# mpeg5/xevd

Hardware: AMD Instinct MI355X
Metric: frames/sec (bit-exact YUV) + achieved HBM GB/s (higher is better)
Workload: dtype s16; 1 GPU; cfg4_main_8k_10b_ra; width=7680, height=4320, bit_depth=10, batches_resident=4, residual_pass_ahead=True, parallelism=1 stream on 1 GPU

## Files before the change

### include/xevd_hip.h

```cpp
#ifndef XEVD_HIP_H
#define XEVD_HIP_H

#include <stddef.h>
#include <stdint.h>

#ifdef __cplusplus
extern "C" {
#endif

#define XGPU_OK                    0
#define XGPU_ERR                  (-1)
#define XGPU_ERR_INVALID_ARGUMENT (-101)
#define XGPU_ERR_OUT_OF_MEMORY    (-102)
#define XGPU_ERR_UNSUPPORTED      (-104)
#define XGPU_ERR_UNEXPECTED       (-105)

#define XGPU_MAX_REFS   17
#define XGPU_PAD_L      144
#define XGPU_PAD_C      72

#define XGPU_MODE_INTRA 0
#define XGPU_MODE_INTER 1
#define XGPU_MODE_SKIP  2
#define XGPU_MODE_DIR   3
// ... 198 lines not shown
int    xgpu_pic_output_device_rois_dev(xgpu_ctx *ctx, int pic, const xgpu_dra_luts *dra, const xgpu_output_format *f, const xgpu_scale_params *sc,
                                       const xgpu_roi_params *rp, const xgpu_roi_bounds *bounds, int box_format, const void *d_boxes, int capacity,
                                       const int *d_count, xgpu_roi_result *d_results, void *d_dst, size_t dst_size, void *stream);
typedef struct xgpu_warp_map { int64_t m[6]; } xgpu_warp_map;
#define XGPU_WARP_CLAMP 0
#define XGPU_WARP_PAD   1
typedef struct xgpu_warp_params { int samples, border; float pad[3]; size_t image_pitch; } xgpu_warp_params;
int    xgpu_warp_from_matrix(const double theta[6], xgpu_warp_map *out);
int    xgpu_warp_from_rotated_box(double cx, double cy, double w, double h, double angle_deg, int dst_w, int dst_h, xgpu_warp_map *out);
int    xgpu_output_warp_check(const xgpu_output_format *f, const xgpu_scale_params *sc, const xgpu_warp_params *wp, const xgpu_warp_map *maps, int n,
                              int width, int height, int bit_depth, int *bad_index);
size_t xgpu_output_warp_size(const xgpu_output_format *f, const xgpu_scale_params *sc, const xgpu_warp_params *wp, int n, int width, int height, int bit_depth);
int    xgpu_pic_output_device_warp(xgpu_ctx *ctx, int pic, const xgpu_dra_luts *dra, const xgpu_output_format *f, const xgpu_scale_params *sc,
                                   const xgpu_warp_params *wp, const xgpu_warp_map *maps, int maps_on_device, int n, int32_t *d_status, void *d_dst,
                                   size_t dst_size, void *stream);
#define XGPU_GRID_Q16_I32 0
#define XGPU_GRID_F32     1
typedef struct xgpu_remap_params { int grid_format, step_log2, samples, border; float pad[3]; size_t grid_pitch, image_pitch; } xgpu_remap_params;
typedef struct xgpu_remap_lens { double fx, fy, cx, cy, k1, k2, p1, p2, k3, nfx, nfy, ncx, ncy; } xgpu_remap_lens;
int    xgpu_remap_grid_dims(int dst_w, int dst_h, int step_log2, int *gw, int *gh);
size_t xgpu_remap_grid_size(const xgpu_scale_params *sc, const xgpu_remap_params *rp, int n);
int    xgpu_output_remap_check(const xgpu_output_format *f, const xgpu_scale_params *sc, const xgpu_remap_params *rp, int n, int width, int height, int bit_depth);
size_t xgpu_output_remap_size(const xgpu_output_format *f, const xgpu_scale_params *sc, const xgpu_remap_params *rp, int n, int width, int height, int bit_depth);
int    xgpu_remap_from_warp(const xgpu_warp_map *map, int dst_w, int dst_h, int step_log2, int32_t *grid);
int    xgpu_remap_from_homography(const double h[9], int dst_w, int dst_h, int step_log2, int32_t *grid);
int    xgpu_remap_from_lens(const xgpu_remap_lens *lens, int dst_w, int dst_h, int step_log2, int32_t *grid);
int    xgpu_pic_output_device_remap(xgpu_ctx *ctx, int pic, const xgpu_dra_luts *dra, const xgpu_output_format *f, const xgpu_scale_params *sc,
                                    const xgpu_remap_params *rp, const void *d_grid, size_t grid_size, int n, void *d_dst, size_t dst_size, void *stream);
#define XGPU_MAX_RUNGS 8
typedef struct xgpu_surface_rung { int width, height; size_t row_pitch; void *d_dst; size_t dst_size; } xgpu_surface_rung;
typedef struct xgpu_ladder_params { int filter; int dst_chroma_loc; } xgpu_ladder_params;
int    xgpu_scale_taps_ex(int n_plane, int subsampling, int siting_half_luma, int n_dst, int dst_subsampling, int dst_siting_half_luma, int filter,
                          int32_t *first, int32_t *count, int16_t *w, int w_stride);
size_t xgpu_output_ladder_rung_size(const xgpu_output_format *f, int rung_width, int rung_height, size_t row_pitch, int bit_depth);
int    xgpu_output_ladder_check(const xgpu_output_format *f, const xgpu_ladder_params *lp, const xgpu_surface_rung *rungs, int n, int width, int height,
                                int bit_depth);
int    xgpu_pic_output_device_ladder(xgpu_ctx *ctx, int pic, const xgpu_dra_luts *dra, const xgpu_output_format *f, const xgpu_ladder_params *lp,
                                     const xgpu_surface_rung *rungs, int n, void *stream);
#define XGPU_SIDE_BLOCKS           0
#define XGPU_SIDE_FLOW_PLANAR      1
#define XGPU_SIDE_FLOW_INTERLEAVED 2
typedef struct xgpu_side_format {
    int layout;
    int dtype;
    int lists;
    int per_poc;
    int crop[4];
    size_t row_pitch;
} xgpu_side_format;
size_t xgpu_side_info_size(const xgpu_side_format *f, int width, int height);
int    xgpu_frame_side_info(xgpu_ctx *ctx, int pic, const xgpu_side_format *f, void *d_dst, size_t dst_size, void *stream);
#define XGPU_RESID_YUV420            0
#define XGPU_RESID_444_PLANAR        1
#define XGPU_RESID_444_INTERLEAVED   2
#define XGPU_RESID_ENERGY            3
typedef struct xgpu_resid_format {
    int layout;
    int dtype;
    int crop[4];
    size_t row_pitch;
} xgpu_resid_format;
size_t xgpu_resid_size(const xgpu_resid_format *f, int width, int height);
int    xgpu_batch_residual(xgpu_ctx *ctx, xgpu_dbatch *db, const xgpu_resid_format *f, void *d_dst, size_t dst_size, void *stream);
#define XGPU_CMP_REF_PIC     0
#define XGPU_CMP_REF_YUV420  1
typedef struct xgpu_compare_ref {
    int kind;
    int pic;
    const void *d_yuv;
    size_t size;
    int dtype;
    size_t row_pitch;
} xgpu_compare_ref;
typedef struct xgpu_compare_params {
    int crop[4];
    int ssim;
    int block_map;
} xgpu_compare_params;
typedef struct xgpu_compare_result {
    uint64_t n[3];
    uint64_t sse[3];
    uint64_t n_diff[3];
    uint64_t first_diff[3];
    uint32_t max_abs[3];
    uint32_t reserved;
    uint64_t ssim_windows[3];
    int64_t  ssim_q30[3];
} xgpu_compare_result;
size_t xgpu_compare_ref_size(const xgpu_compare_ref *r, int width, int height);
size_t xgpu_compare_map_size(const xgpu_compare_params *p, int width, int height);
int    xgpu_compare_check(const xgpu_compare_ref *r, const xgpu_compare_params *p, int width, int height, int bit_depth);
int    xgpu_pic_compare(xgpu_ctx *ctx, int pic, const xgpu_compare_ref *ref, const xgpu_compare_params *p,
                        xgpu_compare_result *d_result, uint64_t *d_map, size_t map_size, void *stream);
typedef struct xgpu_stats_params {
    int crop[4];
    int hist_bits;
    int pctl_e4[2];
    int light;
    int matrix, full_range, chroma_loc, upsample;
    int transfer;
} xgpu_stats_params;
typedef struct xgpu_stats_result {
    uint64_t n[3], sum[3], sum_sq[3];
    uint32_t min[3], max[3];
    uint32_t pctl[3][2];
    uint64_t light_n;
    double   light_sum, light_mean;
    uint32_t light_max_code, light_pctl_code[2], reserved;
    float    light_max, light_pctl[2], reserved2;
} xgpu_stats_result;
size_t xgpu_stats_hist_size(const xgpu_stats_params *p, int bit_depth);
int    xgpu_stats_check(const xgpu_stats_params *p, int width, int height, int bit_depth);
int    xgpu_stats_lin(int transfer, int bit_depth, float lin[4096]);
int    xgpu_pic_stats(xgpu_ctx *ctx, int pic, const xgpu_stats_params *p, xgpu_stats_result *d_result, uint32_t *d_hist, size_t hist_size, void *stream);
int  xgpu_pic_md5(xgpu_ctx *ctx, int pic, const xgpu_dra_luts *dra, uint8_t digest[3][16]);
int  xgpu_pic_download_padded(xgpu_ctx *ctx, int pic, int16_t *buf_y, int16_t *buf_u, int16_t *buf_v);
int  xgpu_pic_upload_padded(xgpu_ctx *ctx, int pic, const int16_t *buf_y, const int16_t *buf_u, const int16_t *buf_v);

int  xgpu_frame_begin(xgpu_ctx *ctx, const xgpu_frame_params *fp);
int  xgpu_batch_create(xgpu_ctx *ctx, const xgpu_cu_batch *b, xgpu_dbatch **out);
int  xgpu_batch_wait_upload(xgpu_ctx *ctx, xgpu_dbatch *db);
int  xgpu_batch_dmvr_mvs(xgpu_ctx *ctx, xgpu_dbatch *db, int16_t *mv, int n);
int  xgpu_set_builder_threads(xgpu_ctx *ctx, int n);
#define XGPU_BATCH_INFO_COUNT 8
int  xgpu_batch_info(xgpu_ctx *ctx, const xgpu_dbatch *db, int info[XGPU_BATCH_INFO_COUNT]);
void xgpu_batch_destroy(xgpu_ctx *ctx, xgpu_dbatch *db);
int  xgpu_batch_prepare(xgpu_ctx *ctx, xgpu_dbatch *db);
int  xgpu_batch_recon(xgpu_ctx *ctx, xgpu_dbatch *db);
int  xgpu_batch_recon_ahead(xgpu_ctx *ctx, xgpu_dbatch *db, xgpu_dbatch *next);
int  xgpu_deblock(xgpu_ctx *ctx);
int  xgpu_alf(xgpu_ctx *ctx, const xgpu_alf_params *ap);
int  xgpu_pad(xgpu_ctx *ctx);
int  xgpu_frame_end(xgpu_ctx *ctx);

enum { XGPU_K_ITDQ = 0, XGPU_K_INTER = 1, XGPU_K_DBK_V = 2, XGPU_K_DBK_H = 3, XGPU_K_PAD = 4, XGPU_K_INTRA = 5,
       XGPU_K_ALF = 6, XGPU_K_AFFINE = 7, XGPU_K_DMVR = 8, XGPU_K_COUNT = 9 };
int  xgpu_timing_enable(xgpu_ctx *ctx, int on);
int  xgpu_timing_reset(xgpu_ctx *ctx);
int  xgpu_timing_get(xgpu_ctx *ctx, double ms[XGPU_K_COUNT], long long launches[XGPU_K_COUNT]);
int  xgpu_measure_copy_bw(xgpu_ctx *ctx, size_t bytes, int iters, double *gbps);

int xgpu_test_mc_l(xgpu_ctx *ctx, const int16_t *ref_plane, int plane_w, int plane_h, int ref_x, int ref_y,
                   int has_dx, int has_dy, int gmv_x, int gmv_y, int16_t *pred, int w, int h, int bit_depth);
int xgpu_test_mc_c(xgpu_ctx *ctx, const int16_t *ref_plane, int plane_w, int plane_h, int ref_x, int ref_y,
                   int has_dx, int has_dy, int gmv_x, int gmv_y, int16_t *pred, int w, int h, int bit_depth);
int xgpu_test_recon(xgpu_ctx *ctx, const int16_t *coef, const int16_t *pred, int is_coef, int cuw, int cuh, int s_rec, int16_t *rec, int bit_depth);
int xgpu_test_dbk(xgpu_ctx *ctx, int16_t *plane, int pw, int ph, int x, int y, int st, int hor, int bit_depth);
int xgpu_test_dbk_chroma(xgpu_ctx *ctx, int16_t *u, int16_t *v, int pw, int ph, int x, int y, int st_u, int st_v, int hor, int bit_depth);
int xgpu_test_batch_resid(xgpu_ctx *ctx, xgpu_dbatch *db, int16_t *resid);
#define XGPU_TEST_BUILD_DIGESTS 13
int xgpu_test_build_batch(const xgpu_seq_params *sp, const xgpu_cu_batch *b, int threads, uint64_t digest[XGPU_TEST_BUILD_DIGESTS], int info[XGPU_BATCH_INFO_COUNT], double *ms);
int xgpu_test_itdq(xgpu_ctx *ctx, int16_t *coef, int n_blocks, int log2w, int log2h, const uint8_t *qp, int bit_depth);
int xgpu_test_itdq_ex(xgpu_ctx *ctx, int16_t *coef, int n_blocks, int log2w, int log2h, const uint8_t *qp, int bit_depth, int tr_v, int tr_h, int log2s);
int xgpu_test_scale_taps_device(xgpu_ctx *ctx, int n_plane, int subsampling, int siting_half_luma, int n_dst, int filter, int32_t *first, int32_t *count,
                                int16_t *w, int w_stride);

#ifdef __cplusplus
}
#endif
#endif
```

### xevd_amd/abi.py

```python
import ctypes as C
import os

import numpy as np

HERE = os.path.dirname(os.path.abspath(__file__))
LIB_PATH = os.path.join(HERE, "libxevd_hip.so")

XGPU_MAX_REFS = 17
PAD_L, PAD_C = 144, 72
MODE_INTRA, MODE_INTER, MODE_SKIP, MODE_DIR = 0, 1, 2, 3
K_NAMES = ["itdq", "inter", "dbk_v", "dbk_h", "pad", "intra", "alf", "affine", "dmvr"]
K_COUNT = 9


class SeqParams(C.Structure):
    _fields_ = [
        ("device", C.c_int), ("width", C.c_int), ("height", C.c_int),
        ("bit_depth_luma", C.c_int), ("bit_depth_chroma", C.c_int), ("chroma_format_idc", C.c_int),
        ("log2_ctu", C.c_int), ("tool_iqt", C.c_int), ("tool_admvp", C.c_int), ("tool_addb", C.c_int),
        ("tool_alf", C.c_int), ("max_pics", C.c_int),
        ("chroma_qp_table", C.POINTER(C.c_int8) * 2),
        ("tool_eipd", C.c_int),
    ]

# ... 561 lines not shown
    cb.pred_mode = _ptr(keep["pred_mode"], C.c_uint8)
    cb.refi, cb.mv = _ptr(keep["refi"], C.c_int8), _ptr(keep["mv"], C.c_int16)
    cb.qp, cb.cbf, cb.ipm = _ptr(keep["qp"], C.c_uint8), _ptr(keep["cbf"], C.c_uint8), _ptr(keep["ipm"], C.c_uint8)
    if keep["cbf_sub"] is not None:
        cb.cbf_sub = _ptr(keep["cbf_sub"], C.c_uint16)
    if keep["ats"] is not None:
        cb.ats = _ptr(keep["ats"], C.c_uint8)
    if keep["ats_inter"] is not None:
        cb.ats_inter = _ptr(keep["ats_inter"], C.c_uint8)
    if keep["affine"] is not None:
        cb.affine, cb.affine_mv = _ptr(keep["affine"], C.c_uint8), _ptr(keep["affine_mv"], C.c_int16)
    if keep["dmvr"] is not None:
        cb.dmvr = _ptr(keep["dmvr"], C.c_uint8)
    if keep["tree"] is not None:
        cb.tree = _ptr(keep["tree"], C.c_uint8)
    cb.coef_off, cb.coef = _ptr(keep["coef_off"], C.c_uint32), _ptr(keep["coef"], C.c_int16)
    cb.n_coef = len(keep["coef"])
    cb.n_ctu = len(keep["ctu_cu_start"]) - 1
    cb.ctu_cu_start = _ptr(keep["ctu_cu_start"], C.c_uint32)
    cb.constrained_intra_pred = int(b.get("constrained_intra_pred", 0) or 0)
    cb.htdf_slice_qp = int(b.get("htdf_slice_qp", 0) or 0)
    if b.get("tiles") is not None:
        keep["tiles"] = make_tile_grid(b["tiles"])
        cb.tiles = C.pointer(keep["tiles"])
    return cb, keep


def make_seq_params(width, height, bit_depth=8, log2_ctu=6, device=0, iqt=0, admvp=0, addb=0, alf=0, max_pics=4,
                    bit_depth_chroma=None, eipd=0):
    sp = SeqParams()
    sp.device, sp.width, sp.height = device, width, height
    sp.bit_depth_luma = bit_depth
    sp.bit_depth_chroma = bit_depth if bit_depth_chroma is None else bit_depth_chroma
    sp.chroma_format_idc = 1
    sp.log2_ctu = log2_ctu
    sp.tool_iqt, sp.tool_admvp, sp.tool_addb, sp.tool_alf = iqt, admvp, addb, alf
    sp.max_pics = max_pics
    sp.tool_eipd = eipd
    return sp


_EXPORTS = {
    "xgpu_open": (C.c_int, [C.POINTER(SeqParams), C.POINTER(C.c_void_p)]),
    "xgpu_close": (None, [C.c_void_p]),
    "xgpu_sync": (C.c_int, [C.c_void_p]),
    "xgpu_last_error": (C.c_char_p, [C.c_void_p]),
    "xgpu_version": (C.c_char_p, []),
    "xgpu_pic_alloc": (C.c_int, [C.c_void_p]),
    "xgpu_pic_free": (C.c_int, [C.c_void_p, C.c_int]),
    "xgpu_pic_upload": (C.c_int, [C.c_void_p, C.c_int, C.c_void_p, C.c_int, C.c_void_p, C.c_void_p, C.c_int]),
    "xgpu_pic_download": (C.c_int, [C.c_void_p, C.c_int, C.c_void_p, C.c_int, C.c_void_p, C.c_void_p, C.c_int]),
    "xgpu_pic_output_size": (C.c_size_t, [C.c_void_p, C.c_int, C.c_int, C.c_int, C.c_int, C.c_int]),
    "xgpu_pic_output": (C.c_int, [C.c_void_p, C.c_int, C.c_void_p, C.c_int, C.c_int, C.c_int, C.c_int, C.c_int, C.c_void_p, C.c_size_t]),
    "xgpu_pic_output_async": (C.c_int, [C.c_void_p, C.c_int, C.c_void_p, C.c_int, C.c_int, C.c_int, C.c_int, C.c_int, C.c_void_p, C.c_size_t, C.POINTER(C.c_int)]),
    "xgpu_pic_output_wait": (C.c_int, [C.c_void_p, C.c_int]),
    "xgpu_pic_md5": (C.c_int, [C.c_void_p, C.c_int, C.c_void_p, C.c_void_p]),
    "xgpu_output_format_size": (C.c_size_t, [C.POINTER(OutputFormat), C.c_int, C.c_int, C.c_int]),
    "xgpu_pic_output_device_size": (C.c_size_t, [C.c_void_p, C.POINTER(OutputFormat)]),
    "xgpu_pic_output_device": (C.c_int, [C.c_void_p, C.c_int, C.c_void_p, C.POINTER(OutputFormat), C.c_void_p, C.c_size_t, C.c_void_p]),
    "xgpu_output_coeffs": (C.c_int, [C.POINTER(OutputFormat), C.c_int, C.POINTER(C.c_int32), C.POINTER(C.c_int), C.POINTER(C.c_float)]),
    "xgpu_colour_tables": (C.c_int, [C.POINTER(OutputFormat), C.POINTER(ColourTransform), C.c_int, C.POINTER(ColourTables)]),
    "xgpu_pic_output_device_cm": (C.c_int, [C.c_void_p, C.c_int, C.c_void_p, C.POINTER(OutputFormat), C.POINTER(ColourTransform), C.c_void_p, C.c_size_t, C.c_void_p]),
    "xgpu_scale_taps": (C.c_int, [C.c_int] * 5 + [C.POINTER(C.c_int32), C.POINTER(C.c_int32), C.POINTER(C.c_int16), C.c_int]),
    "xgpu_output_scaled_size": (C.c_size_t, [C.POINTER(OutputFormat), C.POINTER(ScaleParams), C.c_int, C.c_int, C.c_int]),
    "xgpu_output_scaled_check": (C.c_int, [C.POINTER(OutputFormat), C.POINTER(ScaleParams), C.c_int, C.c_int, C.c_int]),
    "xgpu_pic_output_device_scaled": (C.c_int, [C.c_void_p, C.c_int, C.c_void_p, C.POINTER(OutputFormat), C.POINTER(ScaleParams), C.c_void_p, C.c_size_t, C.c_void_p]),
    "xgpu_scale_taps_ex": (C.c_int, [C.c_int] * 7 + [C.POINTER(C.c_int32), C.POINTER(C.c_int32), C.POINTER(C.c_int16), C.c_int]),
    "xgpu_output_ladder_rung_size": (C.c_size_t, [C.POINTER(OutputFormat), C.c_int, C.c_int, C.c_size_t, C.c_int]),
    "xgpu_output_ladder_check": (C.c_int, [C.POINTER(OutputFormat), C.POINTER(LadderParams), C.POINTER(SurfaceRung), C.c_int, C.c_int, C.c_int, C.c_int]),
    "xgpu_pic_output_device_ladder": (C.c_int, [C.c_void_p, C.c_int, C.c_void_p, C.POINTER(OutputFormat), C.POINTER(LadderParams), C.POINTER(SurfaceRung), C.c_int,
                                                C.c_void_p]),
    "xgpu_roi_inner": (C.c_int, [C.POINTER(Roi), C.POINTER(ScaleParams), C.c_int, C.POINTER(C.c_int)]),
    "xgpu_output_rois_check": (C.c_int, [C.POINTER(OutputFormat), C.POINTER(ScaleParams), C.POINTER(RoiParams), C.POINTER(Roi), C.c_int, C.c_int, C.c_int, C.c_int,
                                         C.POINTER(C.c_int)]),
    "xgpu_output_rois_size": (C.c_size_t, [C.POINTER(OutputFormat), C.POINTER(ScaleParams), C.POINTER(RoiParams), C.POINTER(Roi), C.c_int, C.c_int, C.c_int, C.c_int]),
    "xgpu_pic_output_device_rois": (C.c_int, [C.c_void_p, C.c_int, C.c_void_p, C.POINTER(OutputFormat), C.POINTER(ScaleParams), C.POINTER(RoiParams), C.POINTER(Roi),
                                              C.c_int, C.c_void_p, C.c_size_t, C.c_void_p]),
    "xgpu_output_scaled_cm_check": (C.c_int, [C.POINTER(OutputFormat), C.POINTER(ScaleParams), C.POINTER(ColourTransform), C.c_int, C.c_int, C.c_int]),
    "xgpu_pic_output_device_scaled_cm": (C.c_int, [C.c_void_p, C.c_int, C.c_void_p, C.POINTER(OutputFormat), C.POINTER(ScaleParams), C.POINTER(ColourTransform),
                                                   C.c_void_p, C.c_size_t, C.c_void_p]),
    "xgpu_pic_output_device_rois_cm": (C.c_int, [C.c_void_p, C.c_int, C.c_void_p, C.POINTER(OutputFormat), C.POINTER(ScaleParams), C.POINTER(RoiParams), C.POINTER(Roi),
                                                 C.c_int, C.POINTER(ColourTransform), C.c_void_p, C.c_size_t, C.c_void_p]),
    "xgpu_output_scaled_lin_check": (C.c_int, [C.POINTER(OutputFormat), C.POINTER(ScaleParams), C.POINTER(ColourTransform), C.c_int, C.c_int, C.c_int]),
    "xgpu_output_rois_lin_check": (C.c_int, [C.POINTER(OutputFormat), C.POINTER(ScaleParams), C.POINTER(RoiParams), C.POINTER(Roi), C.c_int, C.POINTER(ColourTransform),
                                             C.c_int, C.c_int, C.c_int, C.POINTER(C.c_int)]),
    "xgpu_pic_output_device_scaled_lin": (C.c_int, [C.c_void_p, C.c_int, C.c_void_p, C.POINTER(OutputFormat), C.POINTER(ScaleParams), C.POINTER(ColourTransform),
                                                    C.c_void_p, C.c_size_t, C.c_void_p]),
    "xgpu_pic_output_device_rois_lin": (C.c_int, [C.c_void_p, C.c_int, C.c_void_p, C.POINTER(OutputFormat), C.POINTER(ScaleParams), C.POINTER(RoiParams), C.POINTER(Roi),
                                                  C.c_int, C.POINTER(ColourTransform), C.c_void_p, C.c_size_t, C.c_void_p]),
    "xgpu_roi_snap": (C.c_int, [C.c_int, C.c_void_p, C.c_int, C.c_int, C.POINTER(Roi)]),
    "xgpu_output_rois_dev_check": (C.c_int, [C.POINTER(OutputFormat), C.POINTER(ScaleParams), C.POINTER(RoiParams), C.POINTER(RoiBounds)] + [C.c_int] * 5),
    "xgpu_output_rois_dev_size": (C.c_size_t, [C.POINTER(OutputFormat), C.POINTER(ScaleParams), C.POINTER(RoiParams), C.POINTER(RoiBounds)] + [C.c_int] * 5),
    "xgpu_pic_output_device_rois_dev": (C.c_int, [C.c_void_p, C.c_int, C.c_void_p, C.POINTER(OutputFormat), C.POINTER(ScaleParams), C.POINTER(RoiParams),
                                                  C.POINTER(RoiBounds), C.c_int, C.c_void_p, C.c_int, C.c_void_p, C.c_void_p, C.c_void_p, C.c_size_t, C.c_void_p]),
    "xgpu_warp_from_matrix": (C.c_int, [C.POINTER(C.c_double), C.POINTER(WarpMap)]),
    "xgpu_warp_from_rotated_box": (C.c_int, [C.c_double] * 5 + [C.c_int, C.c_int, C.POINTER(WarpMap)]),
    "xgpu_output_warp_check": (C.c_int, [C.POINTER(OutputFormat), C.POINTER(ScaleParams), C.POINTER(WarpParams), C.POINTER(WarpMap), C.c_int, C.c_int, C.c_int, C.c_int,
                                         C.POINTER(C.c_int)]),
    "xgpu_output_warp_size": (C.c_size_t, [C.POINTER(OutputFormat), C.POINTER(ScaleParams), C.POINTER(WarpParams), C.c_int, C.c_int, C.c_int, C.c_int]),
    "xgpu_pic_output_device_warp": (C.c_int, [C.c_void_p, C.c_int, C.c_void_p, C.POINTER(OutputFormat), C.POINTER(ScaleParams), C.POINTER(WarpParams), C.c_void_p,
                                              C.c_int, C.c_int, C.c_void_p, C.c_void_p, C.c_size_t, C.c_void_p]),
    "xgpu_remap_grid_dims": (C.c_int, [C.c_int, C.c_int, C.c_int, C.POINTER(C.c_int), C.POINTER(C.c_int)]),
    "xgpu_remap_grid_size": (C.c_size_t, [C.POINTER(ScaleParams), C.POINTER(RemapParams), C.c_int]),
    "xgpu_output_remap_check": (C.c_int, [C.POINTER(OutputFormat), C.POINTER(ScaleParams), C.POINTER(RemapParams), C.c_int, C.c_int, C.c_int, C.c_int]),
    "xgpu_output_remap_size": (C.c_size_t, [C.POINTER(OutputFormat), C.POINTER(ScaleParams), C.POINTER(RemapParams), C.c_int, C.c_int, C.c_int, C.c_int]),
    "xgpu_remap_from_warp": (C.c_int, [C.POINTER(WarpMap), C.c_int, C.c_int, C.c_int, C.POINTER(C.c_int32)]),
    "xgpu_remap_from_homography": (C.c_int, [C.POINTER(C.c_double), C.c_int, C.c_int, C.c_int, C.POINTER(C.c_int32)]),
    "xgpu_remap_from_lens": (C.c_int, [C.POINTER(RemapLens), C.c_int, C.c_int, C.c_int, C.POINTER(C.c_int32)]),
    "xgpu_pic_output_device_remap": (C.c_int, [C.c_void_p, C.c_int, C.c_void_p, C.POINTER(OutputFormat), C.POINTER(ScaleParams), C.POINTER(RemapParams), C.c_void_p,
                                               C.c_size_t, C.c_int, C.c_void_p, C.c_size_t, C.c_void_p]),
    "xgpu_side_info_size": (C.c_size_t, [C.POINTER(SideFormat), C.c_int, C.c_int]),
    "xgpu_frame_side_info": (C.c_int, [C.c_void_p, C.c_int, C.POINTER(SideFormat), C.c_void_p, C.c_size_t, C.c_void_p]),
    "xgpu_resid_size": (C.c_size_t, [C.POINTER(ResidFormat), C.c_int, C.c_int]),
    "xgpu_batch_residual": (C.c_int, [C.c_void_p, C.c_void_p, C.POINTER(ResidFormat), C.c_void_p, C.c_size_t, C.c_void_p]),
    "xgpu_compare_ref_size": (C.c_size_t, [C.POINTER(CompareRef), C.c_int, C.c_int]),
    "xgpu_compare_map_size": (C.c_size_t, [C.POINTER(CompareParams), C.c_int, C.c_int]),
    "xgpu_compare_check": (C.c_int, [C.POINTER(CompareRef), C.POINTER(CompareParams), C.c_int, C.c_int, C.c_int]),
    "xgpu_pic_compare": (C.c_int, [C.c_void_p, C.c_int, C.POINTER(CompareRef), C.POINTER(CompareParams), C.c_void_p, C.c_void_p, C.c_size_t, C.c_void_p]),
    "xgpu_stats_hist_size": (C.c_size_t, [C.POINTER(StatsParams), C.c_int]),
    "xgpu_stats_check": (C.c_int, [C.POINTER(StatsParams), C.c_int, C.c_int, C.c_int]),
    "xgpu_stats_lin": (C.c_int, [C.c_int, C.c_int, C.POINTER(C.c_float)]),
    "xgpu_pic_stats": (C.c_int, [C.c_void_p, C.c_int, C.POINTER(StatsParams), C.c_void_p, C.c_void_p, C.c_size_t, C.c_void_p]),
    "xgpu_host_alloc": (C.c_int, [C.c_void_p, C.c_size_t, C.POINTER(C.c_void_p)]),
    "xgpu_host_free": (None, [C.c_void_p, C.c_void_p]),
    "xgpu_batch_wait_upload": (C.c_int, [C.c_void_p, C.c_void_p]),
    "xgpu_set_builder_threads": (C.c_int, [C.c_void_p, C.c_int]),
    "xgpu_batch_prepare": (C.c_int, [C.c_void_p, C.c_void_p]),
    "xgpu_batch_info": (C.c_int, [C.c_void_p, C.c_void_p, C.POINTER(C.c_int)]),
    "xgpu_batch_dmvr_mvs": (C.c_int, [C.c_void_p, C.c_void_p, C.c_void_p, C.c_int]),
    "xgpu_pic_download_padded": (C.c_int, [C.c_void_p, C.c_int, C.c_void_p, C.c_void_p, C.c_void_p]),
    "xgpu_pic_upload_padded": (C.c_int, [C.c_void_p, C.c_int, C.c_void_p, C.c_void_p, C.c_void_p]),
    "xgpu_frame_begin": (C.c_int, [C.c_void_p, C.POINTER(FrameParams)]),
    "xgpu_batch_create": (C.c_int, [C.c_void_p, C.POINTER(CuBatch), C.POINTER(C.c_void_p)]),
    "xgpu_batch_destroy": (None, [C.c_void_p, C.c_void_p]),
    "xgpu_batch_recon": (C.c_int, [C.c_void_p, C.c_void_p]),
    "xgpu_batch_recon_ahead": (C.c_int, [C.c_void_p, C.c_void_p, C.c_void_p]),
    "xgpu_deblock": (C.c_int, [C.c_void_p]),
    "xgpu_alf": (C.c_int, [C.c_void_p, C.POINTER(AlfParams)]),
    "xgpu_pad": (C.c_int, [C.c_void_p]),
    "xgpu_frame_end": (C.c_int, [C.c_void_p]),
    "xgpu_timing_enable": (C.c_int, [C.c_void_p, C.c_int]),
    "xgpu_timing_reset": (C.c_int, [C.c_void_p]),
    "xgpu_timing_get": (C.c_int, [C.c_void_p, C.POINTER(C.c_double), C.POINTER(C.c_longlong)]),
    "xgpu_measure_copy_bw": (C.c_int, [C.c_void_p, C.c_size_t, C.c_int, C.POINTER(C.c_double)]),
    "xgpu_test_mc_l": (C.c_int, [C.c_void_p, C.c_void_p] + [C.c_int] * 8 + [C.c_void_p] + [C.c_int] * 3),
    "xgpu_test_mc_c": (C.c_int, [C.c_void_p, C.c_void_p] + [C.c_int] * 8 + [C.c_void_p] + [C.c_int] * 3),
    "xgpu_test_batch_resid": (C.c_int, [C.c_void_p, C.c_void_p, C.c_void_p]),
    "xgpu_test_build_batch": (C.c_int, [C.c_void_p, C.c_void_p, C.c_int, C.POINTER(C.c_uint64), C.POINTER(C.c_int), C.POINTER(C.c_double)]),
    "xgpu_test_recon": (C.c_int, [C.c_void_p, C.c_void_p, C.c_void_p] + [C.c_int] * 4 + [C.c_void_p, C.c_int]),
    "xgpu_test_dbk": (C.c_int, [C.c_void_p, C.c_void_p] + [C.c_int] * 7),
    "xgpu_test_dbk_chroma": (C.c_int, [C.c_void_p, C.c_void_p, C.c_void_p] + [C.c_int] * 8),
    "xgpu_test_itdq": (C.c_int, [C.c_void_p, C.c_void_p, C.c_int, C.c_int, C.c_int, C.c_void_p, C.c_int]),
    "xgpu_test_itdq_ex": (C.c_int, [C.c_void_p, C.c_void_p, C.c_int, C.c_int, C.c_int, C.c_void_p, C.c_int, C.c_int, C.c_int, C.c_int]),
    "xgpu_test_scale_taps_device": (C.c_int, [C.c_void_p] + [C.c_int] * 5 + [C.POINTER(C.c_int32), C.POINTER(C.c_int32), C.POINTER(C.c_int16), C.c_int]),
}

_lib = None


def exported_names():
    return sorted(_EXPORTS)


def _share_torch_hip_runtime():
    import importlib.util
    import sys
    if "torch" in sys.modules:
        return
    spec = importlib.util.find_spec("torch")
    if spec is None or not spec.submodule_search_locations:
        return
    rt = os.path.join(list(spec.submodule_search_locations)[0], "lib", "libamdhip64.so")
    if os.path.exists(rt):
        C.CDLL(rt, mode=C.RTLD_GLOBAL)


def load():
    global _lib
    if _lib is None:
        _share_torch_hip_runtime()
        if not os.path.exists(LIB_PATH):
            raise RuntimeError(
                f"{LIB_PATH} is missing: build it with `python -c 'import __graft_entry__ as g; g.build()'` "
                "(hipcc --offload-arch=gfx950).  xevd_amd has no CPU fallback.")
        lib = C.CDLL(LIB_PATH)
        for name, (res, args) in _EXPORTS.items():
            fn = getattr(lib, name)
            fn.restype, fn.argtypes = res, args
        _lib = lib
    return _lib
```

### xevd_amd/csrc/itdq_body.h

```cpp
#pragma once
#include "xgpu_internal.h"
#include <type_traits>

typedef short v2s __attribute__((ext_vector_type(2)));

static __constant__ uint32_t k_tmp[2730];
__host__ __device__ constexpr int tmp_base(int log2n) { return log2n == 1 ? 0 : log2n == 2 ? 2 : log2n == 3 ? 10 : log2n == 4 ? 42 : log2n == 5 ? 170 : 682; }

static __constant__ uint32_t k_atsp[2][680];
__host__ __device__ constexpr int atsp_base(int log2n) { return log2n == 2 ? 0 : log2n == 3 ? 8 : log2n == 4 ? 40 : 168; }

static void upload_transform_tables_tu(const int *tm, const int16_t *ats, hipStream_t s)
{
    static uint32_t apk[2][680];
    for (int t = 0; t < 2; t++) {
        int src = 0;
        for (int l = 2; l <= 5; l++) {
            const int N = 1 << l, dst = atsp_base(l);
            for (int k2 = 0; k2 < N / 2; k2++)
                for (int n = 0; n < N; n++)
                    apk[t][dst + k2 * N + n] = (uint32_t)(uint16_t)ats[t * 1360 + src + (2 * k2) * N + n] |
                                               ((uint32_t)(uint16_t)ats[t * 1360 + src + (2 * k2 + 1) * N + n] << 16);
            src += N * N;
        }
    }
    (void)hipMemcpyToSymbolAsync(HIP_SYMBOL(k_atsp), apk, sizeof(apk), 0, hipMemcpyHostToDevice, s);
    static uint32_t packed[2730];
    int src = 0;
    for (int l = 1; l <= 6; l++) {
        const int N = 1 << l, dst = tmp_base(l);
        for (int k2 = 0; k2 < N / 2; k2++)
            for (int n = 0; n < N; n++)
                packed[dst + k2 * N + n] = (uint32_t)(uint16_t)(int16_t)tm[src + (2 * k2) * N + n] |
                                           ((uint32_t)(uint16_t)(int16_t)tm[src + (2 * k2 + 1) * N + n] << 16);
        src += N * N;
    }
    (void)hipMemcpyToSymbolAsync(HIP_SYMBOL(k_tmp), packed, sizeof(packed), 0, hipMemcpyHostToDevice, s);
    (void)hipStreamSynchronize(s);
}

__device__ __forceinline__ int clip16(int v) { return min(max(v, -32768), 32767); }
__device__ __forceinline__ int dot2(uint32_t a, uint32_t b, int c)
{
    return __builtin_amdgcn_sdot2(__builtin_bit_cast(v2s, a), __builtin_bit_cast(v2s, b), c, false);
}
__device__ __forceinline__ int mad24(int a, int b, int c)
{
    int r;
    asm("v_mad_i32_i24 %0, %1, %2, %3" : "=v"(r) : "v"(a), "v"(b), "v"(c));
    return r;
}
__device__ __forceinline__ uint32_t pack16(int lo, int hi) { return (uint32_t)(uint16_t)lo | ((uint32_t)hi << 16); }

__host__ __device__ constexpr int itdq_group(int lw, int lh)
{
    const int W = 1 << lw, H = 1 << lh;
    const int l1 = W * (H > 16 ? H / 16 : 1), l2 = H * (W > 16 ? W / 16 : 1);
    return 256 / (l1 > l2 ? l1 : l2);
}

#define ITDQ_PLANES_DWORDS 4608
#define ITDQ_LDS_DWORDS (ITDQ_PLANES_DWORDS + 2048)
#define ITDQ_MAX_G 32
#define ITDQ_TB_DWORDS (4 * ITDQ_MAX_G)

typedef uint32_t itq_v2 __attribute__((ext_vector_type(2)));
typedef uint32_t itq_v4 __attribute__((ext_vector_type(4)));
typedef itq_v2 __attribute__((aligned(4))) itq_v2_u;
typedef itq_v4 __attribute__((aligned(2))) itq_v4_u;
typedef itq_v2 __attribute__((aligned(2))) itq_v2_s;
template <typename T> __device__ __forceinline__ T itq_any() { T v; asm volatile("" : "=v"(v)); return v; }
static_assert(sizeof(TbRec) == 8, "a TbRec is fetched as one 8-byte load: off | log2w, log2h, qp, log2s");
__device__ __forceinline__ void itq_rec_if(itq_v2 &v, const TbRec *p, bool on) { if (on) v = *(const itq_v2_u *)p; }
__device__ __forceinline__ int rec_qp(itq_v2 r) { return (int)((r.y >> 16) & 0xFF); }
__device__ __forceinline__ int rec_log2s(itq_v2 r) { return (int)(r.y >> 24); }

template <bool ODD, bool IQT>
struct ItdqScale {
    int mul, cmax, shift, offset;
    __device__ __forceinline__ ItdqScale(int qp, int bd, int lwh)
    {
        shift = bd - 9 + (lwh >> 1) + (ODD ? 8 : 0);
        offset = shift == 0 ? 0 : 1 << (shift - 1);
        const int q6 = (int)(((uint32_t)qp * 171u) >> 10), sidx = qp - 6 * q6;
        constexpr uint64_t scale = 40ull | 45ull << 8 | 51ull << 16 | 57ull << 24 | 64ull << 32 | (uint64_t)(IQT ? 72 : 71) << 40;
        const int sbase = (int)((scale >> (8 * sidx)) & 0xFF);
        mul = sbase << q6;
        cmax = (1 << 23) >> q6;
    }
    __device__ __forceinline__ int operator()(int c) const
    {
        if constexpr (!ODD) {
            const int held = min(max(c, -cmax), cmax);
            return clip16(mad24(held, mul, offset) >> shift);
        }
        const long long l = ((long long)(c * (ODD ? 181 : 1)) * mul + offset) >> shift;
        return (int)min(max(l, -32768ll), 32767ll);
    }
};

template <int G, int LX>
__device__ __forceinline__ uint32_t wave_masks(const uint32_t *s_m, int t)
{
    constexpr int X = 1 << LX, PER = 64 / X > 1 ? 64 / X : 1, N = G < PER ? G : PER;
    const int p0 = __builtin_amdgcn_readfirstlane(((t & ~63) % (G * X)) >> LX);
    static_assert(G * X >= 64 ? (G % N == 0) : (64 % (G * X) == 0 && N == G), "the wave's TBs are entries [p0, p0 + N)");
    uint32_t m = 0;
#pragma unroll
    for (int i = 0; i < N; i++) m |= s_m[p0 + i];
    return (uint32_t)__builtin_amdgcn_readfirstlane((int)m);
}

template <int L>
__device__ __forceinline__ const uint32_t *itdq_matrix(int tr) { return (tr == TR_DCT2 || L < 2 || L > 5) ? k_tmp + tmp_base(L) : k_atsp[tr - 1] + atsp_base(L); }

template <int LW, int LH, bool IQT>
__device__ __forceinline__ void itdq_small(const ItdqArgs &a, const TbWave wv)
{
    constexpr int W = 1 << LW, H = 1 << LH, S = W * H;
    static_assert(S <= 16 && itdq_group(LW, LH) <= 256, "one TB per lane");
    const int p = threadIdx.x;
    if (p >= wv.count) return;
    const itq_v2 rec = *(const itq_v2_u *)(a.tbs + wv.first + p);
    const uint32_t *tmh = itdq_matrix<LH>(wv.tr_v), *tmw = itdq_matrix<LW>(wv.tr_h);
    const bool s16_mid = IQT || wv.tr_v != TR_DCT2 || wv.tr_h != TR_DCT2;
    uint32_t raw[S / 2];
    if constexpr (S == 4) { const itq_v2 v = *(const itq_v2_s *)(a.coef + rec.x); raw[0] = v.x; raw[1] = v.y; }
    else {
#pragma unroll
        for (int i = 0; i < S / 8; i++) {
            const itq_v4 v = *(const itq_v4_u *)(a.coef + rec.x + 8 * i);
            raw[4 * i] = v.x; raw[4 * i + 1] = v.y; raw[4 * i + 2] = v.z; raw[4 * i + 3] = v.w;
        }
    }
    const ItdqScale<(LW + LH) & 1, IQT> dq(rec_qp(rec), a.bd, LW + LH);
    int d[S];
#pragma unroll
    for (int i = 0; i < S / 2; i++) {
        d[2 * i] = 0; d[2 * i + 1] = 0;
        if (raw[i] != 0) { d[2 * i] = dq((int16_t)(raw[i] & 0xFFFF)); d[2 * i + 1] = dq((int16_t)(raw[i] >> 16)); }
    }
    uint32_t mh[H][W / 2], ml[H][W / 2];
#pragma unroll
    for (int jj = 0; jj < W / 2; jj++) {
        int acc[2][H];
#pragma unroll
        for (int e = 0; e < 2; e++) {
#pragma unroll
            for (int n = 0; n < H; n++) acc[e][n] = 0;
#pragma unroll
            for (int k2 = 0; k2 < H / 2; k2++) {
                const uint32_t vp = pack16(d[(2 * k2) * W + 2 * jj + e], d[(2 * k2 + 1) * W + 2 * jj + e]);
#pragma unroll
                for (int n = 0; n < H; n++) acc[e][n] = dot2(tmh[k2 * H + n], vp, acc[e][n]);
            }
        }
#pragma unroll
        for (int n = 0; n < H; n++) {
            if (s16_mid) mh[n][jj] = pack16(clip16((acc[0][n] + 64) >> 7), clip16((acc[1][n] + 64) >> 7));
            else if constexpr (!IQT) {
                mh[n][jj] = pack16(acc[0][n] >> 15, acc[1][n] >> 15);
                ml[n][jj] = pack16(acc[0][n] & 0x7FFF, acc[1][n] & 0x7FFF);
            }
        }
    }
    const int shift2 = s16_mid ? 12 - (a.bd - 8) : 7 + 12 - (a.bd - 8);
    uint32_t out[S / 2];
#pragma unroll
    for (int r = 0; r < H; r++) {
        int res[W];
        if (s16_mid) {
            int s[W];
#pragma unroll
            for (int n = 0; n < W; n++) s[n] = 1 << (shift2 - 1);
#pragma unroll
            for (int k2 = 0; k2 < W / 2; k2++) {
#pragma unroll
                for (int n = 0; n < W; n++) s[n] = dot2(tmw[k2 * W + n], mh[r][k2], s[n]);
            }
#pragma unroll
            for (int n = 0; n < W; n++) res[n] = clip16(s[n] >> shift2);
        } else if constexpr (!IQT) {
            int sh[W], sl[W];
#pragma unroll
            for (int n = 0; n < W; n++) { sh[n] = 0; sl[n] = 0; }
#pragma unroll
            for (int k2 = 0; k2 < W / 2; k2++) {
#pragma unroll
                for (int n = 0; n < W; n++) { sh[n] = dot2(tmw[k2 * W + n], mh[r][k2], sh[n]); sl[n] = dot2(tmw[k2 * W + n], ml[r][k2], sl[n]); }
            }
            const long long add = 1ll << (shift2 - 1);
#pragma unroll
            for (int n = 0; n < W; n++) {
                const long long s = (long long)sh[n] * 32768 + sl[n] + add;
                res[n] = (int)min(max(s >> shift2, -32768ll), 32767ll);
            }
        }
#pragma unroll
        for (int n = 0; n < W; n += 2) out[(r * W + n) / 2] = pack16(res[n], res[n + 1]);
    }
    int16_t *dst = a.resid + rec.x;
    if constexpr (S == 4) { itq_v2 v; v.x = out[0]; v.y = out[1]; *(itq_v2_s *)dst = v; }
    else {
#pragma unroll
        for (int i = 0; i < S / 8; i++) {
            itq_v4 v; v.x = out[4 * i]; v.y = out[4 * i + 1]; v.z = out[4 * i + 2]; v.w = out[4 * i + 3];
            *(itq_v4_u *)(dst + 8 * i) = v;
        }
    }
}

template <int LW, int LH, bool IQT>
__device__ __forceinline__ void itdq_item(const ItdqArgs &a, const TbWave wv, uint32_t *lds, uint32_t *s_tb)
{
    constexpr int W = 1 << LW, H = 1 << LH;
    constexpr int N1 = H > 16 ? 16 : H, C1 = H / N1;
    constexpr int N2 = W > 16 ? 16 : W, C2 = W / N2;
    constexpr int G = itdq_group(LW, LH);
    constexpr int RS = W / 2 + 1;
    constexpr int PLANE = G * H * RS;
    constexpr bool UNI1 = (G * W) % 64 == 0, UNI2 = (G * H) % 64 == 0;
    static_assert(2 * PLANE <= ITDQ_PLANES_DWORDS && G * W * H <= 4096 && G <= ITDQ_MAX_G, "LDS budget");
    constexpr int PLANES_DWORDS = IQT ? ITDQ_PLANES_DWORDS / 2 : ITDQ_PLANES_DWORDS;
    constexpr bool RMASK = H >= 16, CMASK = W >= 16;
    uint32_t *s_rm = s_tb, *s_cm = s_tb + ITDQ_MAX_G, *s_rec = s_tb + 2 * ITDQ_MAX_G;
    const int t = threadIdx.x;

    constexpr int S = W * H, UN = S >= 8 ? 8 : 4, NU = G * S / UN, NR = (NU + 255) / 256;
    typedef typename std::conditional<UN == 8, itq_v4, itq_v2>::type cvec;
    bool on[NR];
    int up[NR], uo[NR];
    itq_v2 rec[NR];
#pragma unroll
    for (int r = 0; r < NR; r++) {
        const int u = t + 256 * r;
        up[r] = (u * UN) / S; uo[r] = (u * UN) % S;
        on[r] = (NU % 256 == 0 || u < NU) && up[r] < wv.count;
        rec[r] = itq_any<itq_v2>();
        itq_rec_if(rec[r], a.tbs + wv.first + up[r], on[r]);
    }
    if (RMASK || CMASK) {
        if (t < G) { s_rm[t] = 0; s_cm[t] = 0; }
        __syncthreads();
    }
    const uint32_t *tmh = itdq_matrix<LH>(wv.tr_v), *tmw = itdq_matrix<LW>(wv.tr_h);
    const bool s16_mid = IQT || wv.tr_v != TR_DCT2 || wv.tr_h != TR_DCT2;
    asm volatile("" :: "s"(tmh), "s"(tmw));
    int16_t *ldsh = (int16_t *)lds;
    int16_t *ldsl = (int16_t *)(lds + PLANE);
    uint32_t *ldsc = lds + PLANES_DWORDS;
    cvec cv[NR];
#pragma unroll
    for (int r = 0; r < NR; r++) {
        cv[r] = itq_any<cvec>();
        if (on[r]) {
            const int16_t *src = a.coef + rec[r].x + ((uo[r] >> LW) << rec_log2s(rec[r])) + (uo[r] & (W - 1));
            if constexpr (UN == 8) cv[r] = *(const itq_v4_u *)src; else cv[r] = *(const itq_v2_s *)src;
        }
    }
#pragma unroll
    for (int r = 0; r < NR; r++) {
        if (!on[r]) continue;
        const int p = up[r], o = uo[r];
        const ItdqScale<(LW + LH) & 1, IQT> dq(rec_qp(rec[r]), a.bd, LW + LH);
        if (o == 0) { s_rec[2 * p] = rec[r].x; s_rec[2 * p + 1] = rec[r].y; }
        uint32_t raw[UN / 2];
#pragma unroll
        for (int i = 0; i < UN / 2; i++) raw[i] = cv[r][i];
#pragma unroll
        for (int i = 0; i < UN / 2; i++) {
            if (raw[i] == 0) continue;
            raw[i] = pack16(dq((int16_t)(raw[i] & 0xFFFF)), dq((int16_t)(raw[i] >> 16)));
            if (RMASK) atomicOr(&s_rm[p], 1u << ((o + 2 * i) >> (LW + 1)));
            if (CMASK) atomicOr(&s_cm[p], 1u << (((o + 2 * i) & (W - 1)) >> 1));
        }
#pragma unroll
        for (int i = 0; i < UN / 2; i++) ldsc[(p * S + o) / 2 + i] = raw[i];
    }
    __syncthreads();

    uint32_t rows1 = 0;
    if (RMASK) rows1 = wave_masks<G, LW>(s_rm, t);
    if (t < G * W * C1) {
        const int idx = t % (G * W);
        int chunk = t / (G * W);
        if (UNI1) chunk = __builtin_amdgcn_readfirstlane(chunk);
        const int p = idx >> LW, j = idx & (W - 1);
        const bool valid = p < wv.count;
        const uint32_t vmask = valid ? 0xFFFFFFFFu : 0u;
        const int16_t *src = (const int16_t *)ldsc + p * (W * H) + j;

        int acc[N1];
#pragma unroll
        for (int n = 0; n < N1; n++) acc[n] = 0;
        if (RMASK) {
            for (uint32_t m = rows1; m; m &= m - 1) {
                const int k2 = __builtin_ctz(m);
                const uint32_t vp = pack16(src[(2 * k2) * W], src[(2 * k2 + 1) * W]) & vmask;
                const uint32_t *row = tmh + k2 * H + chunk * N1;
#pragma unroll
                for (int n = 0; n < N1; n++) acc[n] = dot2(row[n], vp, acc[n]);
            }
        } else {
            for (int k2 = 0; k2 < H / 2; k2++) {
                const uint32_t vp = pack16(src[(2 * k2) * W], src[(2 * k2 + 1) * W]) & vmask;
                if (__ballot(vp != 0) == 0) continue;
                const uint32_t *row = tmh + k2 * H + chunk * N1;
#pragma unroll
                for (int n = 0; n < N1; n++) acc[n] = dot2(row[n], vp, acc[n]);
            }
        }
        const int base = (p * H + chunk * N1) * (2 * RS) + j;
        if (CMASK && !(valid && ((s_cm[p] >> (j >> 1)) & 1))) {
        } else if (s16_mid) {
#pragma unroll
            for (int n = 0; n < N1; n++) ldsh[base + n * (2 * RS)] = (int16_t)clip16((acc[n] + 64) >> 7);
        } else {
#pragma unroll
            for (int n = 0; n < N1; n++) {
                ldsh[base + n * (2 * RS)] = (int16_t)(acc[n] >> 15);
                ldsl[base + n * (2 * RS)] = (int16_t)(acc[n] & 0x7FFF);
            }
        }
    }
    __syncthreads();

    uint32_t cols2 = 0;
    if (CMASK) cols2 = wave_masks<G, LH>(s_cm, t);
    if (t < G * H * C2) {
        const int idx = t % (G * H);
        int chunk = t / (G * H);
        if (UNI2) chunk = __builtin_amdgcn_readfirstlane(chunk);
        const int p = idx >> LH, r = idx & (H - 1);
        if (p >= wv.count) return;
        const uint32_t own = CMASK ? s_cm[p] : 0xFFFFFFFFu;
        itq_v2 tb;
        tb.x = s_rec[2 * p]; tb.y = s_rec[2 * p + 1];
        const int shift2 = s16_mid ? 12 - (a.bd - 8) : 7 + 12 - (a.bd - 8);
        const uint32_t *inh = lds + (p * H + r) * RS;
        const uint32_t *inl = inh + PLANE;
        int res[N2];
        if (s16_mid) {
            int s[N2];
#pragma unroll
            for (int n = 0; n < N2; n++) s[n] = 1 << (shift2 - 1);
            if (CMASK) {
                for (uint32_t m = cols2; m; m &= m - 1) {
                    const int k2 = __builtin_ctz(m);
                    const uint32_t vp = inh[k2] & (0u - ((own >> k2) & 1));
                    const uint32_t *row = tmw + k2 * W + chunk * N2;
#pragma unroll
                    for (int n = 0; n < N2; n++) s[n] = dot2(row[n], vp, s[n]);
                }
            } else {
                for (int k2 = 0; k2 < W / 2; k2++) {
                    const uint32_t vp = inh[k2];
                    if (__ballot(vp != 0) == 0) continue;
                    const uint32_t *row = tmw + k2 * W + chunk * N2;
#pragma unroll
                    for (int n = 0; n < N2; n++) s[n] = dot2(row[n], vp, s[n]);
                }
            }
#pragma unroll
            for (int n = 0; n < N2; n++) res[n] = clip16(s[n] >> shift2);
        } else {
            int sh[N2], sl[N2];
#pragma unroll
            for (int n = 0; n < N2; n++) { sh[n] = 0; sl[n] = 0; }
            if (CMASK) {
                for (uint32_t m = cols2; m; m &= m - 1) {
                    const int k2 = __builtin_ctz(m);
                    const uint32_t mine = 0u - ((own >> k2) & 1);
                    const uint32_t vh = inh[k2] & mine, vl = inl[k2] & mine;
                    const uint32_t *row = tmw + k2 * W + chunk * N2;
#pragma unroll
                    for (int n = 0; n < N2; n++) { sh[n] = dot2(row[n], vh, sh[n]); sl[n] = dot2(row[n], vl, sl[n]); }
                }
            } else {
                for (int k2 = 0; k2 < W / 2; k2++) {
                    const uint32_t vh = inh[k2], vl = inl[k2];
                    if (__ballot((vh | vl) != 0) == 0) continue;
                    const uint32_t *row = tmw + k2 * W + chunk * N2;
#pragma unroll
                    for (int n = 0; n < N2; n++) { sh[n] = dot2(row[n], vh, sh[n]); sl[n] = dot2(row[n], vl, sl[n]); }
                }
            }
            const long long add = 1ll << (shift2 - 1);
#pragma unroll
            for (int n = 0; n < N2; n++) {
                const long long s = (long long)sh[n] * 32768 + sl[n] + add;
                res[n] = (int)min(max(s >> shift2, -32768ll), 32767ll);
            }
        }
        int16_t *out = a.resid + tb.x + (r << rec_log2s(tb)) + chunk * N2;
        if constexpr (N2 >= 8) {
#pragma unroll
            for (int n = 0; n < N2; n += 8) {
                uint4 v;
                v.x = pack16(res[n + 0], res[n + 1]);
                v.y = pack16(res[n + 2], res[n + 3]);
                v.z = pack16(res[n + 4], res[n + 5]);
                v.w = pack16(res[n + 6], res[n + 7]);
                *(uint4 *)(out + n) = v;
            }
        } else if constexpr (N2 == 4) {
            uint2 v;
            v.x = pack16(res[0], res[1]);
            v.y = pack16(res[2], res[3]);
            *(uint2 *)out = v;
        } else {
            *(uint32_t *)out = pack16(res[0], res[1]);
        }
    }
}

template <bool IQT>
__device__ __forceinline__ void itdq_dispatch(const ItdqArgs &a, int wi, uint32_t *lds, uint32_t *s_tb)
{
    static_assert(sizeof(TbWave) == 12 && alignof(TbWave) == 4, "TbWave is read as three dwords");
    const uint32_t *w = (const uint32_t *)(a.waves + wi);
    const uint32_t w0 = w[0], w1 = w[1], w2 = w[2];
    TbWave wv;
    wv.first = w0; wv.count = (uint16_t)(w1 & 0xFFFF); wv.log2w = (uint8_t)(w1 >> 16); wv.log2h = (uint8_t)(w1 >> 24); wv.tr_v = (uint8_t)w2; wv.tr_h = (uint8_t)(w2 >> 8);
#define CASE(lw, lh) case (lw) * 8 + (lh): if constexpr ((lw) + (lh) <= 4) itdq_small<lw, lh, IQT>(a, wv); else itdq_item<lw, lh, IQT>(a, wv, lds, s_tb); break;
#define ROW(lw) CASE(lw, 1) CASE(lw, 2) CASE(lw, 3) CASE(lw, 4) CASE(lw, 5) CASE(lw, 6)
    switch (wv.log2w * 8 + wv.log2h) {
        ROW(1) ROW(2) ROW(3) ROW(4) ROW(5) ROW(6)
        default: break;
    }
#undef ROW
#undef CASE
}
```

### xevd_amd/csrc/k_intra.hip

```cpp
#include "xgpu_internal.h"
#include "itdq_body.h"

#include <type_traits>
#include "intra_pred.h"

#define INTRA_WAVES 8


__constant__ uint8_t k_htdf_tbl[5][16] = {
    { 0, 0, 2,  6, 10, 14, 19, 23, 28, 32,  36,  41,  45,  49,  53,  57 },
    { 0, 0, 5, 12, 20, 29, 38, 47, 56, 65,  73,  82,  90,  98, 107, 115 },
    { 0, 0, 1,  4,  9, 16, 24, 32, 41, 50,  59,  68,  77,  86,  94, 103 },
    { 0, 0, 3,  9, 19, 32, 47, 64, 81, 99, 117, 135, 154, 179, 205, 230 },
    { 0, 0, 0,  2,  6, 11, 18, 27, 38, 51,  64,  96, 128, 160, 192, 224 },
};
#define HTDF_EXT (66 * 66)

template <bool HTDF> struct IntraLds { static constexpr int WAVE = (HTDF && HTDF_EXT > 3 * NB_LEN) ? HTDF_EXT : 3 * NB_LEN; };

#ifdef INTRA_PROFILE
__device__ uint32_t g_intra_prof[8 * 64];
#define ISTAMP(k) do { if (DEP && t == 0 && item >= INTRA_PROFILE && item < INTRA_PROFILE + 64) g_intra_prof[8 * (item - INTRA_PROFILE) + (k)] = (uint32_t)clock64(); } while (0)
#else
#define ISTAMP(k)
// ... 462 lines not shown
            else                 filter_tiles(std::integral_constant<int, 2>{}, std::integral_constant<int, 2>{});
        }
        ISTAMP(4);
        if (DEP) {
            asm volatile("s_waitcnt vmcnt(0)" ::: "memory");
            ISTAMP(5);
            if (t == 0) __hip_atomic_store(&a.done[item], a.epoch, __ATOMIC_RELAXED, __HIP_MEMORY_SCOPE_AGENT);
        }
        wave_lds_sync();
        if (!DEP) break;
        item = uni(q0.x);
        if (item == 0xFFFFFFFFu) break;
    }
}

#define SB_C0 71
#define SB_UR 144
#define SB_LEN (SB_UR + 72)
#define SMALL_GROUPS (4 * INTRA_WAVES)
__device__ __forceinline__ void intra_small_body(const IntraArgs &a, uint32_t block, int16_t *s_nb_)
{
    int16_t (*s_nb)[3][SB_LEN] = (int16_t (*)[3][SB_LEN])s_nb_;
    const int g = threadIdx.x >> 4, t = threadIdx.x & 15;
    const uint32_t k = block * SMALL_GROUPS + (uint32_t)g;
    if (k >= (uint32_t)a.n_small) return;
    const uint32_t item = (uint32_t)(a.first + a.count - a.n_small) + k;
    int16_t (*nb)[SB_LEN] = s_nb[g];
    const int mid = 1 << (a.bd_l - 1), maxv = (1 << a.bd_l) - 1;
    const uint4 *rec = (const uint4 *)&a.list[item];
    const uint4 q0 = rec[0], q1 = rec[1], q2 = rec[2];
    const uint32_t nflags = q0.y, avail_ul = nflags & 1;
    const int lrf = (int)((nflags >> 23) & 3);
    const uint64_t avail_up = (uint64_t)q0.z | ((lrf & 2) ? 0ull : (uint64_t)q0.w << 32);
    const uint64_t avail_le = (uint64_t)q1.x | ((uint64_t)q1.y << 32);
    const uint32_t gg = q2.x, m = q2.y, ipm = q2.z, coef_off = q2.w;
    const int cu_x = gg & 0xFFFF, cu_y = gg >> 16;
    const int lw = m & 0xFF, lh = (m >> 8) & 0xFF, cbf = (m >> 16) & 0xFF;
    const int mode_l = ipm & 0xFF, mode_c = (ipm >> 8) & 0xFF;
    const int cw = 1 << lw, chh = 1 << lh, scuw = cw >> 2, nscu = scuw * (chh >> 2), cwc = cw >> 1;
    const uint32_t off_u = coef_off + ((cbf & 1) ? (uint32_t)(cw * chh) : 0u);
    const uint32_t off_v = off_u + ((cbf & 2) ? (uint32_t)(cwc * (chh >> 1)) : 0u);
    const bool has = t < nscu;
    const int lx = (t & (scuw - 1)) << 2, ly = (t >> (lw - 2)) << 2;

    uint2 rl[4] = { { 0, 0 }, { 0, 0 }, { 0, 0 }, { 0, 0 } };
    uint32_t rc[2][2] = { { 0, 0 }, { 0, 0 } };
    if (has) {
        if (cbf & 1)
#pragma unroll
            for (int r = 0; r < 4; r++) rl[r] = *(const uint2 *)(a.resid + coef_off + (ly + r) * cw + lx);
#pragma unroll
        for (int c = 1; c < 3; c++)
            if ((cbf >> c) & 1)
#pragma unroll
                for (int r = 0; r < 2; r++) rc[c - 1][r] = *(const uint32_t *)(a.resid + (c == 1 ? off_u : off_v) + ((ly >> 1) + r) * cwc + (lx >> 1));
    }

#pragma unroll
    for (int c = 0; c < 3; c++) {
        const int16_t *plane = c == 0 ? a.cur_y : (c == 1 ? a.cur_u : a.cur_v);
        const int s = c ? a.s_c : a.s_l, sh = c ? 1 : 0, ush = c ? 1 : 2;
        const int16_t *org = plane + (cu_y >> sh) * s + (cu_x >> sh);
        const int n = (cw + chh) >> sh;
        const int eu = min(2 * t, n - 2), e0 = min(t, n - 1), e1 = min(t + 16, n - 1);
        const uint32_t vu = *(const uint32_t *)(org - s + eu);
        const uint32_t v0 = (uint16_t)org[e0 * s - 1], v1 = (uint16_t)org[e1 * s - 1], vc = (uint16_t)org[-s - 1];
        const uint32_t midp = (uint32_t)mid * 0x10001u;
        if (2 * t < n) *(uint32_t *)&nb[c][SB_C0 + 1 + 2 * t] = ((avail_up >> (eu >> ush)) & 1) ? vu : midp;
        if (t < n) nb[c][SB_C0 - 1 - t] = (int16_t)(((avail_le >> (e0 >> ush)) & 1) ? v0 : (uint32_t)mid);
        if (t + 16 < n) nb[c][SB_C0 - 1 - (t + 16)] = (int16_t)(((avail_le >> (e1 >> ush)) & 1) ? v1 : (uint32_t)mid);
        if (t == 0) nb[c][SB_C0] = (int16_t)(avail_ul ? vc : (uint32_t)mid);
        if (n > 32) {
            for (int e = 2 * t + 32; e < n; e += 32)
                *(uint32_t *)&nb[c][SB_C0 + 1 + e] = ((avail_up >> (e >> ush)) & 1) ? *(const uint32_t *)(org - s + e) : midp;
            for (int e = t + 32; e < n; e += 16)
                nb[c][SB_C0 - 1 - e] = ((avail_le >> (e >> ush)) & 1) ? org[e * s - 1] : (int16_t)mid;
        }
    }
    wave_lds_sync();
#pragma unroll
    for (int c = 0; c < 3; c++) {
        const int mode = c ? mode_c : mode_l;
        const int w = c ? cw >> 1 : cw, h = c ? chh >> 1 : chh;
        if (mode == 0) {
            int acc = 0;
            for (int e = t; e < w + h; e += 16) acc += e < h ? nb[c][SB_C0 - 1 - e] : nb[c][SB_C0 + 1 + e - h];
            acc = row_sum16(acc);
            if (t == 0) nb[c][NB_DC] = (int16_t)((acc + w) >> ((c ? lw - 1 : lw) + 1));
        } else if (mode == 4) {
            for (int e = t; e < w + h; e += 16) nb[c][SB_UR + e] = (int16_t)((nb[c][SB_C0 + 1 + e] + nb[c][SB_C0 - 1 - e]) >> 1);
        }
    }
    wave_lds_sync();
    if (!has) return;
    const int x = cu_x + lx, y = cu_y + ly;
    int pl[4][4], pc[2][2][2];
    int vl[7], vc[2][3];
    nb_fetch<7, SB_C0, SB_UR>(nb[0], mode_l, lx, ly, vl);
    nb_fetch<3, SB_C0, SB_UR>(nb[1], mode_c, lx >> 1, ly >> 1, vc[0]);
    nb_fetch<3, SB_C0, SB_UR>(nb[2], mode_c, lx >> 1, ly >> 1, vc[1]);
#pragma unroll
    for (int md = 0; md < 5; md++) {
        if (md == mode_l)
#pragma unroll
            for (int r = 0; r < 4; r++)
#pragma unroll
                for (int q = 0; q < 4; q++) pl[r][q] = vl[nb_sel(md, r, q, 3)];
        if (md == mode_c)
#pragma unroll
            for (int c = 0; c < 2; c++)
#pragma unroll
                for (int r = 0; r < 2; r++)
#pragma unroll
                    for (int q = 0; q < 2; q++) pc[c][r][q] = vc[c][nb_sel(md, r, q, 1)];
    }
    int16_t *dy = a.cur_y + y * a.s_l + x;
    const int coff = (y >> 1) * a.s_c + (x >> 1);
    if (!(nflags & 32u))
#pragma unroll
        for (int r = 0; r < 4; r++) {
            const uint32_t o0 = recon2i(pack2i(pl[r][0], pl[r][1]), (cbf & 1) ? rl[r].x : 0u, maxv), o1 = recon2i(pack2i(pl[r][2], pl[r][3]), (cbf & 1) ? rl[r].y : 0u, maxv);
            *(uint2 *)(dy + r * a.s_l) = make_uint2(o0, o1);
        }
    if (!(nflags & 64u))
#pragma unroll
        for (int c = 1; c < 3; c++) {
            int16_t *d = (c == 1 ? a.cur_u : a.cur_v) + coff;
#pragma unroll
            for (int r = 0; r < 2; r++)
                *(uint32_t *)(d + r * a.s_c) = recon2i(pack2i(pc[c - 1][r][0], pc[c - 1][r][1]), ((cbf >> c) & 1) ? rc[c - 1][r] : 0u, maxv);
        }
}

__global__ __launch_bounds__(64 * INTRA_WAVES) void k_intra_l1(const IntraArgs a, uint32_t big)
{
    constexpr int BIG_LDS = INTRA_WAVES * IntraLds<false>::WAVE, SMALL_LDS = SMALL_GROUPS * 3 * SB_LEN;
    __shared__ __attribute__((aligned(16))) int16_t s_nb[BIG_LDS > SMALL_LDS ? BIG_LDS : SMALL_LDS];
    if (blockIdx.x < big) {
        IntraArgs b = a;
        b.count = a.count - a.n_small;
        intra_body<false, 0, false, false, INTRA_WAVES>(b, blockIdx.x, s_nb, nullptr);
    } else intra_small_body(a, blockIdx.x - big, s_nb);
}

template <bool DEP, int EIPD, bool IBC, bool HTDF>
__global__ __launch_bounds__(64 * INTRA_WAVES) void k_intra(const IntraArgs a)
{
    __shared__ __attribute__((aligned(16))) int16_t s_nb[INTRA_WAVES * IntraLds<HTDF>::WAVE];
    __shared__ uint32_t s_chunk;
    intra_body<DEP, EIPD, IBC, HTDF, INTRA_WAVES>(a, blockIdx.x, s_nb, &s_chunk);
}

#define FUSED_WAVES 4
template <int EIPD, bool IBC, bool IQT>
__global__ __launch_bounds__(64 * FUSED_WAVES) void k_intra_itdq(const IntraArgs a, const ItdqArgs r, uint32_t n_intra_wg, uint64_t rate)
{
    constexpr int ITDQ_DW = (IQT ? ITDQ_LDS_DWORDS - ITDQ_PLANES_DWORDS / 2 : ITDQ_LDS_DWORDS) + ITDQ_TB_DWORDS, INTRA_DW = (FUSED_WAVES * IntraLds<false>::WAVE + 1) / 2 + 4;
    __shared__ __attribute__((aligned(16))) uint32_t raw[ITDQ_DW > INTRA_DW ? ITDQ_DW : INTRA_DW];
    const uint32_t before = min(n_intra_wg, (uint32_t)(((uint64_t)blockIdx.x * rate) >> 32)), after = min(n_intra_wg, (uint32_t)(((uint64_t)(blockIdx.x + 1) * rate) >> 32));
    if (after > before) {
        intra_body<true, EIPD, IBC, false, FUSED_WAVES>(a, blockIdx.x, (int16_t *)raw, raw + INTRA_DW - 1);
    } else {
        const int wi = (int)(blockIdx.x - before);
        if (wi >= r.n_waves) return;
        itdq_dispatch<IQT>(r, wi, raw, raw + ITDQ_DW - ITDQ_TB_DWORDS);
    }
}

void upload_transform_tables_intra(const int *tm, const int16_t *ats, hipStream_t s) { upload_transform_tables_tu(tm, ats, s); }

int intra_chunk(bool with_itdq) { return with_itdq ? FUSED_WAVES : INTRA_WAVES; }

void launch_intra(xgpu_ctx *c, const IntraArgs &a, bool dep, bool ibc, bool htdf, const ItdqArgs *next, bool right)
{
    right = right && c->sp.tool_eipd;
    if (next) {
        const uint32_t n_wg = (uint32_t)((a.count + FUSED_WAVES - 1) / FUSED_WAVES);
        const dim3 g(n_wg + (uint32_t)next->n_waves), b(64 * FUSED_WAVES);
        const uint32_t span = std::max(n_wg, g.x / 2);
        const uint64_t rate = (((uint64_t)n_wg << 32) + span - 1) / span;
#define LAUNCHF(E, I) do { if (next->iqt) hipLaunchKernelGGL((k_intra_itdq<E, I, true>), g, b, 0, c->stream, a, *next, n_wg, rate); else hipLaunchKernelGGL((k_intra_itdq<E, I, false>), g, b, 0, c->stream, a, *next, n_wg, rate); } while (0)
        if (right) LAUNCHF(2, true);
        else if (c->sp.tool_eipd) { if (ibc) LAUNCHF(1, true); else LAUNCHF(1, false); }
        else                 { if (ibc) LAUNCHF(0, true); else LAUNCHF(0, false); }
#undef LAUNCHF
        return;
    }
    const int per = INTRA_WAVES;
    if (!dep && !right && !htdf && !ibc && !c->sp.tool_eipd && a.n_small >= c->intra_small_min) {
        const uint32_t big = (uint32_t)((a.count - a.n_small + per - 1) / per), small_blocks = (uint32_t)((a.n_small + SMALL_GROUPS - 1) / SMALL_GROUPS);
        hipLaunchKernelGGL(k_intra_l1, dim3(big + small_blocks), dim3(64 * INTRA_WAVES), 0, c->stream, a, big);
        return;
    }
    const int blocks = (a.count + per - 1) / per;
    const dim3 g(blocks), b(64 * INTRA_WAVES);
#define LAUNCH(D, E, I, H) hipLaunchKernelGGL((k_intra<D, E, I, H>), g, b, 0, c->stream, a)
    if (right) { if (dep) LAUNCH(true, 2, true, true); else LAUNCH(false, 2, true, true); }
    else if (htdf) {
        if (c->sp.tool_eipd) { if (dep) LAUNCH(true, 1, true, true); else LAUNCH(false, 1, true, true); }
        else                 { if (dep) LAUNCH(true, 0, true, true); else LAUNCH(false, 0, true, true); }
    } else if (ibc) {
        if (c->sp.tool_eipd) { if (dep) LAUNCH(true, 1, true, false); else LAUNCH(false, 1, true, false); }
        else                 { if (dep) LAUNCH(true, 0, true, false); else LAUNCH(false, 0, true, false); }
    } else {
        if (c->sp.tool_eipd) { if (dep) LAUNCH(true, 1, false, false); else LAUNCH(false, 1, false, false); }
        else                 { if (dep) LAUNCH(true, 0, false, false); else LAUNCH(false, 0, false, false); }
    }
#undef LAUNCH
#ifdef INTRA_PROFILE
    static int shots = 0;
    if (dep && ++shots == 5) {
        hipStreamSynchronize(c->stream);
        uint32_t h[8 * 64];
        hipMemcpyFromSymbol(h, HIP_SYMBOL(g_intra_prof), sizeof(h));
        for (int i = 0; i < 64; i++)
            fprintf(stderr, "  pos %d start %10u  wait %6u stage %5u (EIPD luma: issue %5u, return %5u | HTDF: to the block loads %5u from stamp 3, block in LDS %5u) plan %5u predict %5u ack %5u\n", INTRA_PROFILE + i, h[8 * i], h[8 * i + 1] - h[8 * i],
                    h[8 * i + 2] - h[8 * i + 1], h[8 * i + 6] - h[8 * i + 1], h[8 * i + 7] - h[8 * i + 6], h[8 * i + 6] - h[8 * i + 3], h[8 * i + 7] - h[8 * i + 6], h[8 * i + 3] - h[8 * i + 2], h[8 * i + 4] - h[8 * i + 3], h[8 * i + 5] - h[8 * i + 4]);
    }
#endif
}
```

### xevd_amd/csrc/xgpu_api.hip

```cpp
#include "xgpu_host.h"

static const int8_t k_chroma_qp_main[58] = { 0, 1, 2, 3, 4, 5, 6, 7, 8, 9, 10, 11, 12, 13, 14, 15, 16, 17, 18, 19, 20, 21, 22, 23, 24, 25, 26, 27, 28, 29,
    29, 30, 31, 32, 33, 34, 35, 36, 37, 37, 38, 39, 40, 40, 41, 42, 43, 44, 45, 46, 47, 48, 49, 50, 51, 52, 53, 54 };
static const int8_t k_chroma_qp_base[58] = {
     0,  1,  2,  3,  4,  5,  6,  7,  8,  9, 10, 11, 12, 13, 14, 15, 16, 17, 18, 19,
    20, 21, 22, 23, 24, 25, 26, 27, 28, 29, 29, 29, 30, 31, 32, 32, 33, 33, 34, 34,
    35, 35, 36, 36, 36, 37, 37, 37, 38, 38, 39, 39, 40, 40, 40, 41, 41, 41 };


const char *xgpu_version(void) { return "xevd_amd 0.1 (gfx950)"; }
const char *xgpu_last_error(const xgpu_ctx *c) { return c ? c->err : "null ctx"; }

void time_begin(xgpu_ctx *c, int k, hipEvent_t *a, hipEvent_t *b)
{
    if (!c->timing) return;
    auto get = [&]() {
        hipEvent_t e;
        if (!c->ev_pool.empty()) { e = c->ev_pool.back(); c->ev_pool.pop_back(); }
        else (void)hipEventCreate(&e);
        return e;
    };
    *a = get(); *b = get();
    (void)hipEventRecord(*a, c->stream);
    (void)k;
}
void time_end(xgpu_ctx *c, int k, hipEvent_t a, hipEvent_t b)
{
    if (!c->timing) return;
    (void)hipEventRecord(b, c->stream);
    c->ev_pending.push_back({ a, b, k });
}
int xgpu_timing_enable(xgpu_ctx *c, int on) { ARGCHK(c, c != NULL); c->timing = on; return XGPU_OK; }
int xgpu_timing_reset(xgpu_ctx *c)
{
    ARGCHK(c, c != NULL);
    HIPCHK(c, hipStreamSynchronize(c->stream));
    for (auto &e : c->ev_pending) { c->ev_pool.push_back(e.a); c->ev_pool.push_back(e.b); }
    c->ev_pending.clear();
    memset(c->t_ms, 0, sizeof(c->t_ms));
    memset(c->t_n, 0, sizeof(c->t_n));
    return XGPU_OK;
}
int xgpu_timing_get(xgpu_ctx *c, double ms[XGPU_K_COUNT], long long n[XGPU_K_COUNT])
{
    ARGCHK(c, c != NULL);
    HIPCHK(c, hipStreamSynchronize(c->stream));
    for (auto &e : c->ev_pending) {
        float t = 0;
        HIPCHK(c, hipEventElapsedTime(&t, e.a, e.b));
        c->t_ms[e.k] += t; c->t_n[e.k]++;
        c->ev_pool.push_back(e.a); c->ev_pool.push_back(e.b);
    }
    c->ev_pending.clear();
    for (int i = 0; i < XGPU_K_COUNT; i++) { ms[i] = c->t_ms[i]; n[i] = c->t_n[i]; }
    return XGPU_OK;
}

static void init_transform_tables(xgpu_ctx *c)
{
    static int tm[5460];
    int o = 0;
    for (int l = 1; l <= 6; l++) {
        const int N = 1 << l;
        for (int k = 0; k < N; k++)
            for (int n = 0; n < N; n++) {
                const double v = k == 0 ? 64.0 : 64.0 * sqrt(2.0) * cos((2 * n + 1) * k * 3.14159265358979323846 / (2.0 * N));
                tm[o++] = (int)(v >= 0 ? floor(v + 0.5) : -floor(-v + 0.5));
            }
    }
    static int16_t ats[2 * 1360];
    for (int t = 0; t < 2; t++) {
        int q = t * 1360;
        for (int l = 2; l <= 5; l++) {
            const int N = 1 << l;
            const double sc = sqrt((double)N) * 64;
            int16_t m[32 * 32];
            for (int k = 0; k < N; k++)
                for (int n = 0; n < N; n++) {
                    const double v = t == 0 ? sin(3.14159265358979323846 * (k + 0.5) * (n + 1) / (N + 0.5)) * sqrt(2.0 / (N + 0.5))
                                            : cos(3.14159265358979323846 * (k + 0.5) * (n + 0.5) / (N + 0.5)) * sqrt(2.0 / (N + 0.5));
                    m[k * N + n] = (int16_t)(sc * v + (v > 0 ? 0.5 : -0.5));
                }
            if (N == 4) {
                const int a = m[0], b = m[1], cc = m[2], d = m[3];
                const int e7[16] = { a, b, cc, b + a,  cc, cc, 0, -cc,  a + b, -a, -cc, b,  b, -(b + a), cc, -a };
                const int e8[16] = { d + cc, b, cc, d,  b, 0, -b, -b,  cc, -b, -d, d + cc,  d, -b, d + cc, -cc };
                for (int i = 0; i < 16; i++) m[i] = (int16_t)(t == 0 ? e7[i] : e8[i]);
            }
            for (int i = 0; i < N * N; i++) ats[q++] = m[i];
        }
    }
    upload_transform_tables(tm, ats, c->stream);
}

int xgpu_open(const xgpu_seq_params *sp, xgpu_ctx **out)
{
    if (!sp || !out) return XGPU_ERR_INVALID_ARGUMENT;
    *out = NULL;
    if (sp->chroma_format_idc != 1) return XGPU_ERR_UNSUPPORTED;
    if (sp->width <= 0 || sp->height <= 0 || (sp->width & 7) || (sp->height & 7)) return XGPU_ERR_INVALID_ARGUMENT;
    if (sp->bit_depth_luma < 8 || sp->bit_depth_luma > 12 || sp->bit_depth_chroma < 8 || sp->bit_depth_chroma > 12) return XGPU_ERR_UNSUPPORTED;
    if (sp->log2_ctu < 5 || sp->log2_ctu > 7) return XGPU_ERR_INVALID_ARGUMENT;
    int ndev = 0;
    if (hipGetDeviceCount(&ndev) != hipSuccess || ndev <= 0 || sp->device < 0 || sp->device >= ndev) return XGPU_ERR_UNEXPECTED;

    xgpu_ctx *c = new xgpu_ctx();
    c->sp = *sp;
    c->sp.chroma_qp_table[0] = c->sp.chroma_qp_table[1] = NULL;
    c->builder_threads = 1;
    c->err[0] = 0; c->timing = 0; c->have_frame = 0; c->side_pic = -1; c->d_maps = NULL; c->d_dra = NULL; c->d_cm = NULL; c->cm_tab = NULL; c->d_ctb_flag = NULL; c->stream = 0; c->up_stream = 0; c->down_stream = 0; c->side_stream = 0; c->after_inter = 0; c->have_after_inter = 0; c->where = 0; c->addb_pending = 0;
    c->fork_ev = c->join_ev = 0;
    c->intra_small_min = getenv("XEVD_HIP_INTRA_SMALL_MIN") ? std::max(1, atoi(getenv("XEVD_HIP_INTRA_SMALL_MIN"))) : 2048;
    c->addb_scalar = getenv("XEVD_HIP_ADDB_SCALAR") != NULL;
    c->dmvr_scalar = getenv("XEVD_HIP_DMVR_SCALAR") != NULL;
    c->split_addb_alf = getenv("XEVD_HIP_SPLIT_ADDB_ALF") != NULL;
    for (int i = 0; i < 2; i++) { c->d_out[i] = NULL; c->out_caps[i] = 0; c->out_ready[i] = c->out_done[i] = 0; c->out_busy[i] = 0; }
    c->d_md5 = NULL; c->md5_ready = 0;
    c->odev_ev[0] = c->odev_ev[1] = 0;
    c->sc_tab = NULL; c->sc_tab_cap = 0; c->sc_mid = NULL; c->sc_mid_cap = 0; c->cmp_part = NULL; c->cmp_part_cap = 0; c->stats_blk = NULL; c->stats_lin_tc = c->stats_lin_bd = -1;
    c->roi_blk = NULL; c->roi_blk_cap = 0;
    c->lad_blk = NULL; c->lad_blk_cap = 0; c->lad_cap = 0;
    for (int i = 0; i < 6; i++) c->sc_key[i] = -1;
    c->out_next = 0;
    memset(c->t_ms, 0, sizeof(c->t_ms)); memset(c->t_n, 0, sizeof(c->t_n));
    const int boff = 6 * (sp->bit_depth_chroma - 8);
    for (int t = 0; t < 2; t++)
        for (int q = -boff; q <= 57; q++)
            c->chroma_qp[t][q + boff] = sp->chroma_qp_table[t] ? sp->chroma_qp_table[t][q + boff] : (int8_t)(q < 0 ? q : (sp->tool_iqt ? k_chroma_qp_main[q] : k_chroma_qp_base[q]));

    auto fail = [&](int code) { xgpu_close(c); return code; };
    if (hipSetDevice(sp->device) != hipSuccess) return fail(XGPU_ERR_UNEXPECTED);
    static const bool blocking = getenv("XEVD_HIP_BLOCKING_SYNC") != NULL && atoi(getenv("XEVD_HIP_BLOCKING_SYNC")) != 0;
    if (blocking) (void)hipSetDeviceFlags(hipDeviceScheduleBlockingSync);
    const unsigned ev_flags = hipEventDisableTiming | (blocking ? hipEventBlockingSync : 0);
    {
        static std::atomic<int> n_ctx(0);
        static const bool no_rot = getenv("XEVD_HIP_NO_QUEUE_ROTATION") != NULL;
        const bool swap = !no_rot && (n_ctx.fetch_add(1) & 1);
        hipStream_t *const order[4] = { swap ? &c->side_stream : &c->stream, &c->up_stream, &c->down_stream, swap ? &c->stream : &c->side_stream };
        for (int i = 0; i < 4; i++)
            if (hipStreamCreateWithFlags(order[i], hipStreamNonBlocking) != hipSuccess) return fail(XGPU_ERR_UNEXPECTED);
    }
    if (hipEventCreateWithFlags(&c->after_inter, hipEventDisableTiming) != hipSuccess) return fail(XGPU_ERR_UNEXPECTED);
    if (hipEventCreateWithFlags(&c->fork_ev, hipEventDisableTiming) != hipSuccess || hipEventCreateWithFlags(&c->join_ev, hipEventDisableTiming) != hipSuccess) return fail(XGPU_ERR_UNEXPECTED);
    for (int i = 0; i < 2; i++)
        if (hipEventCreateWithFlags(&c->out_ready[i], hipEventDisableTiming) != hipSuccess || hipEventCreateWithFlags(&c->out_done[i], ev_flags) != hipSuccess)
            return fail(XGPU_ERR_UNEXPECTED);

    ctx_geometry(c);

    if (hipMalloc((void **)&c->d_maps, sizeof(ScuRec) * (size_t)c->w_scu * c->h_scu) != hipSuccess) return fail(XGPU_ERR_OUT_OF_MEMORY);
    if (hipMemsetAsync(c->d_maps, 0, sizeof(ScuRec) * (size_t)c->w_scu * c->h_scu, c->stream) != hipSuccess) return fail(XGPU_ERR_UNEXPECTED);
    if (hipMalloc((void **)&c->d_ctb_flag, (size_t)c->w_ctu * c->h_ctu + 16) != hipSuccess) return fail(XGPU_ERR_OUT_OF_MEMORY);
    init_transform_tables(c);
    c->pics.resize(1 + std::max(1, std::min(sp->max_pics, 34)));
    for (auto &p : c->pics) { p.base = NULL; p.used = 0; }
    {
        DevPic &p = c->pics[0];
        if (hipMalloc((void **)&p.base, c->pic_elems * sizeof(int16_t)) != hipSuccess) return fail(XGPU_ERR_OUT_OF_MEMORY);
        (void)hipMemsetAsync(p.base, 0, c->pic_elems * sizeof(int16_t), c->stream);
        p.s_l = c->s_l; p.s_c = c->s_c; p.used = 1;
        p.y = p.base + (size_t)XGPU_PAD_L * c->s_l + XGPU_MARGIN_L;
        p.u = p.base + c->off_u + (size_t)XGPU_PAD_C * c->s_c + XGPU_MARGIN_C;
        p.v = p.base + c->off_v + (size_t)XGPU_PAD_C * c->s_c + XGPU_MARGIN_C;
    }
    if (hipStreamSynchronize(c->stream) != hipSuccess) return fail(XGPU_ERR_UNEXPECTED);
    *out = c;
    return XGPU_OK;
}

void xgpu_close(xgpu_ctx *c)
{
    if (!c) return;
    (void)hipSetDevice(c->sp.device);
    if (c->stream) (void)hipStreamSynchronize(c->stream);
    if (c->up_stream) (void)hipStreamSynchronize(c->up_stream);
    if (c->down_stream) (void)hipStreamSynchronize(c->down_stream);
    if (c->side_stream) (void)hipStreamSynchronize(c->side_stream);
    for (auto &p : c->pics) if (p.base) (void)hipFree(p.base);
    if (c->d_maps) (void)hipFree(c->d_maps);
    for (BatchBlock &k : c->pool) block_free(k);
    for (auto &h : c->pinned) (void)hipHostFree(h.p);
    c->pinned.clear();
    c->pool.clear();
    if (c->d_md5) (void)hipFree(c->d_md5);
    if (c->md5_ready) (void)hipEventDestroy(c->md5_ready);
    for (int i = 0; i < 2; i++) if (c->odev_ev[i]) (void)hipEventDestroy(c->odev_ev[i]);
    for (int i = 0; i < 2; i++) { if (c->d_out[i]) (void)hipFree(c->d_out[i]); if (c->out_ready[i]) (void)hipEventDestroy(c->out_ready[i]); if (c->out_done[i]) (void)hipEventDestroy(c->out_done[i]); }
    if (c->d_dra) (void)hipFree(c->d_dra);
    if (c->d_cm) (void)hipFree(c->d_cm);
    delete c->cm_tab;
    if (c->sc_tab) (void)hipFree(c->sc_tab);
    if (c->sc_mid) (void)hipFree(c->sc_mid);
    if (c->cmp_part) (void)hipFree(c->cmp_part);
    if (c->stats_blk) (void)hipFree(c->stats_blk);
    if (c->roi_blk) (void)hipFree(c->roi_blk);
    if (c->lad_blk) (void)hipFree(c->lad_blk);
    if (c->d_ctb_flag) (void)hipFree(c->d_ctb_flag);
    for (auto &e : c->ev_pending) { (void)hipEventDestroy(e.a); (void)hipEventDestroy(e.b); }
    for (auto &e : c->ev_pool) (void)hipEventDestroy(e);
    if (c->stream) (void)hipStreamDestroy(c->stream);
    if (c->up_stream) (void)hipStreamDestroy(c->up_stream);
    if (c->down_stream) (void)hipStreamDestroy(c->down_stream);
    if (c->side_stream) (void)hipStreamDestroy(c->side_stream);
    if (c->after_inter) (void)hipEventDestroy(c->after_inter);
    if (c->fork_ev) (void)hipEventDestroy(c->fork_ev);
    if (c->join_ev) (void)hipEventDestroy(c->join_ev);
    delete c;
}

int xgpu_sync(xgpu_ctx *c)
{
    ARGCHK(c, c != NULL);
    HIPCHK(c, hipStreamSynchronize(c->up_stream));
    HIPCHK(c, hipStreamSynchronize(c->side_stream));
    HIPCHK(c, hipStreamSynchronize(c->stream));
    HIPCHK(c, hipStreamSynchronize(c->down_stream));
    return XGPU_OK;
}

int xgpu_host_alloc(xgpu_ctx *c, size_t bytes, void **out)
{
    ARGCHK(c, c != NULL); ARGCHK(c, out != NULL && bytes > 0);
    *out = NULL;
    HIPCHK(c, hipSetDevice(c->sp.device));
    void *p = NULL;
    if (hipHostMalloc(&p, bytes, hipHostMallocDefault) != hipSuccess) { snprintf(c->err, sizeof(c->err), "host_alloc: cannot pin %zu bytes", bytes); return XGPU_ERR_OUT_OF_MEMORY; }
    std::lock_guard<std::mutex> g(c->pool_mu);
    c->pinned.push_back({ (uint8_t *)p, bytes });
    *out = p;
    return XGPU_OK;
}
void xgpu_host_free(xgpu_ctx *c, void *p)
{
    if (!c || !p) return;
    std::lock_guard<std::mutex> g(c->pool_mu);
    for (size_t i = 0; i < c->pinned.size(); i++)
        if (c->pinned[i].p == (uint8_t *)p) { (void)hipHostFree(p); c->pinned.erase(c->pinned.begin() + (long)i); return; }
}


int xgpu_pic_alloc(xgpu_ctx *c)
{
    ARGCHK(c, c != NULL);
    HIPCHK(c, hipSetDevice(c->sp.device));
    for (size_t i = 1; i < c->pics.size(); i++) {
        DevPic &p = c->pics[i];
        if (p.used) continue;
        if (!p.base) {
            if (hipMalloc((void **)&p.base, c->pic_elems * sizeof(int16_t)) != hipSuccess) {
                snprintf(c->err, sizeof(c->err), "hipMalloc of a %zu-byte picture failed", c->pic_elems * sizeof(int16_t));
                return XGPU_ERR_OUT_OF_MEMORY;
            }
            HIPCHK(c, hipMemsetAsync(p.base, 0, c->pic_elems * sizeof(int16_t), c->stream));
        }
        p.s_l = c->s_l; p.s_c = c->s_c;
        p.y = p.base + (size_t)XGPU_PAD_L * c->s_l + XGPU_MARGIN_L;
        p.u = p.base + c->off_u + (size_t)XGPU_PAD_C * c->s_c + XGPU_MARGIN_C;
        p.v = p.base + c->off_v + (size_t)XGPU_PAD_C * c->s_c + XGPU_MARGIN_C;
        p.used = 1;
        return (int)i - 1;
    }
    snprintf(c->err, sizeof(c->err), "no free picture slot (max_pics=%d)", c->sp.max_pics);
    return XGPU_ERR_OUT_OF_MEMORY;
// ... 170 lines not shown
```

### xevd_amd/csrc/xgpu_internal.h

```cpp
#pragma once
#include <hip/hip_runtime.h>
#include <stdint.h>
#include <stdio.h>
#include <string.h>
#include <condition_variable>
#include <functional>
#include <mutex>
#include <thread>
#include <vector>
#include "../../include/xevd_hip.h"

#define XGPU_MARGIN_L 192
#define XGPU_MARGIN_C 128

struct DevPic {
    int16_t *base;
    int16_t *y, *u, *v;
    int      s_l, s_c;
    int      used;
};

struct __attribute__((aligned(16))) CuRec {
    uint16_t x, y;
    uint8_t  log2w, log2h;
// ... 160 lines not shown
    __host__ __device__ static int tile_end(const uint32_t *m, int i, int n)
    {
        for (int w = (i + 1) >> 5; w < 8; w++) {
            uint32_t v = m[w];
            if (w == ((i + 1) >> 5)) v &= 0xFFFFFFFFu << ((i + 1) & 31);
            if (v) { const int e = (w << 5) + __builtin_ctz(v); return e < n ? e : n; }
        }
        return n;
    }
};

struct DbkArgs {
    int      s_l, s_c;
    int      pic_w, pic_h, w_scu, h_scu;
    int      bd_l, bd_c;
    int      ctu_sh;
    TileMask no_filter;
    const ScuRec *maps;
    uint8_t  st[3][4][64];
};

#define ADDB_LDS_TABLE_BYTES (52 + 52 + 260 + XGPU_MAX_REFS * 2 + 192)
#define ADDB_LDS_TABLE_DWORDS ((ADDB_LDS_TABLE_BYTES + 3) / 4)
struct AddbArgs {
    int      s_l, s_c;
    int      w_scu, h_scu;
    int      bd_l, bd_c, log2_ctu;
    int      alpha_off, beta_off, qp_u_off, qp_v_off;
    TileMask no_filter;
    const ScuRec *maps;
    int8_t   chroma_qp[2 * 96];
    uint8_t  pic_id[XGPU_MAX_REFS * 2];
    uint32_t lds_tables[ADDB_LDS_TABLE_DWORDS];
};

#define ALF_CTB_BITS 8704
struct AlfArgs {
    int      s_l, s_c, pic_w, pic_h, bd, log2_ctu, w_ctu, across_tiles;
    TileMask tiles;
    uint32_t magic_tiles_x;
    int      multi_tile;
    int      pad;
    int      enable[3];
    const uint8_t *ctb_flag;
    int      ctb_in_args;
    uint32_t ctb_bits[ALF_CTB_BITS / 32];
    uint32_t ctab[25 * 4][8];
    uint32_t cchroma[4];
};

struct BatchBlock { uint8_t *d_base; size_t d_cap; void *h_stage; size_t h_cap; hipEvent_t uploaded, done, itdq_done;
                    uint32_t *d_chroma; size_t chroma_cap; };

struct xgpu_dbatch {
    BatchBlock blk;
    int        n_cu, n_ctu, n_tb, n_waves;
    size_t     n_coef;
    CuRec     *d_cus;
    uint32_t  *d_ctu_start;
    uint32_t  *d_owner;
    InterItem *d_inter_items;
    uint32_t  *d_inter_work;
    int        n_inter_work;
    int16_t   *d_coef, *d_resid;
    TbRec     *d_tbs;
    TbWave    *d_waves;
    DmvrItem  *d_dmvr_items;
    int16_t   *d_dmvr_mv;
    int        n_dmvr;
    AffItem   *d_aff_items;
    int16_t   *d_cpmv;
    int        n_aff_eif, n_aff_sub;
    IntraRec  *d_intra;
    uint32_t  *d_intra_deps;
    uint32_t  *d_intra_done;
    int        has_ibc, has_htdf;
    int        order_rl;
    int        has_right;
    TileMask   tile_starts;
    int        tiles_across;
    int        n_intra_l1_small;
    int        n_intra, n_levels, n_intra_deps, n_intra_l1, n_intra_heads;
    uint32_t   intra_epoch, intra_tickets;
    void      *h_stage;
    int        host_only;
    size_t     stage_bytes;
    int        prepared;
    int        upload_waited;
    int        used;
    uint32_t  *h_chroma_cus, *d_chroma_cus;
    int        n_chroma_cus;
};

struct ScaleTabs { size_t off_first[4], off_count[4], off_w[4]; int stride[4]; int capy, capc; };
struct ScaleAxisTab { size_t first, count, w; int stride; };
struct xgpu_ctx {
    xgpu_seq_params sp;
    int8_t          chroma_qp[2][96];
    hipStream_t     stream;
    hipStream_t     up_stream, down_stream;
    hipStream_t     side_stream;
    hipEvent_t      after_inter;
    int             have_after_inter;
    std::mutex      pool_mu;
    struct HostRange { uint8_t *p; size_t n; };
    std::vector<HostRange> pinned;
    int             w_scu, h_scu, w_ctu, h_ctu;
    int             s_l, s_c, rows_l, rows_c;
    size_t          pic_elems, off_u, off_v;
    std::vector<DevPic> pics;
    ScuRec         *d_maps;
    uint8_t        *d_ctb_flag;
    std::vector<BatchBlock> pool;
    uint8_t        *d_out[2];
    uint8_t        *d_md5;
    hipEvent_t      md5_ready;
    size_t          out_caps[2];
    hipEvent_t      out_ready[2], out_done[2];
    int             out_busy[2], out_next;
    int32_t        *d_dra;
    float          *d_cm;
    xgpu_colour_tables_t *cm_tab;
    xgpu_colour_transform cm_key;
    int             cm_bd;
    uint8_t        *sc_tab;
    size_t          sc_tab_cap;
    int             sc_key[6];
    ScaleTabs       sc_host;
    uint16_t       *sc_mid;
    size_t          sc_mid_cap;
    unsigned long long *cmp_part;
    size_t          cmp_part_cap;
    uint8_t        *stats_blk;
    int             stats_lin_tc, stats_lin_bd;
    uint8_t        *roi_blk;
    size_t          roi_blk_cap;
    uint8_t        *lad_blk;
    size_t          lad_blk_cap;
    std::vector<int> lad_key;
    std::vector<uint8_t> lad_host;
    std::vector<uint8_t> lad_sent;
    std::vector<ScaleAxisTab> lad_tabs;
    int             lad_cap;
    hipEvent_t      odev_ev[2];
    xgpu_frame_params fp;
    int             have_frame;
    int             side_pic;
    TileMask        no_dbk;
    hipEvent_t      fork_ev, join_ev;
    int             builder_threads;
    int             pad_done;
    int             where;
    int             order_rl;
    int             intra_small_min;
    int             addb_scalar;
    int             dmvr_scalar;
    int             addb_pending, split_addb_alf;
    AddbArgs        addb_args;
    int             timing;
    struct Ev { hipEvent_t a, b; int k; };
    std::vector<Ev> ev_pending;
    std::vector<hipEvent_t> ev_pool;
    double          t_ms[XGPU_K_COUNT];
    long long       t_n[XGPU_K_COUNT];
    char            err[256];
};

class WorkPool {
public:
    ~WorkPool() { { std::lock_guard<std::mutex> g(mu); stop = true; } cv.notify_all(); for (std::thread &t : th) t.join(); }
    template <class F> void run(int n, F &&f)
    {
        if (n <= 1) { f(0); return; }
        while ((int)th.size() < n - 1) { const int idx = (int)th.size(); th.emplace_back([this, idx]() { worker(idx); }); }
        const std::function<void(int)> fn = [&f](int k) { f(k); };
        { std::lock_guard<std::mutex> g(mu); job = &fn; want = n - 1; left = n - 1; gen++; }
        cv.notify_all();
        f(0);
        std::unique_lock<std::mutex> g(mu);
        done_cv.wait(g, [this]() { return left == 0; });
        job = nullptr;
    }
private:
    void worker(int idx)
    {
        uint64_t seen = 0;
        for (;;) {
            const std::function<void(int)> *fn = nullptr;
            {
                std::unique_lock<std::mutex> g(mu);
                cv.wait(g, [&]() { return stop || gen != seen; });
                if (stop) return;
                seen = gen;
                if (idx < want) fn = job;
            }
            if (!fn) continue;
            (*fn)(idx + 1);
            std::lock_guard<std::mutex> g(mu);
            if (--left == 0) done_cv.notify_one();
        }
    }
    std::vector<std::thread> th;
    std::mutex mu;
    std::condition_variable cv, done_cv;
    const std::function<void(int)> *job = nullptr;
    int want = 0, left = 0;
    uint64_t gen = 0;
    bool stop = false;
};

void launch_itdq(xgpu_ctx *c, const ItdqArgs &a, hipStream_t s);
void launch_inter(xgpu_ctx *c, const InterArgs &a);
void launch_test_recon(xgpu_ctx *c, const int16_t *coef, const int16_t *pred, int is_coef, int cuw, int cuh, int16_t *rec, int s_rec, int bd);
void launch_test_dbk(xgpu_ctx *c, int16_t *buf, int16_t *buf_v, int st, int st_v, int stride, int bd, int hor, int chroma);
void launch_intra(xgpu_ctx *c, const IntraArgs &a, bool dep, bool ibc, bool htdf, const ItdqArgs *next, bool right = false);
int  intra_chunk(bool with_itdq);
void launch_affine(xgpu_ctx *c, const AffineArgs &a, hipStream_t s);
void launch_dmvr(xgpu_ctx *c, const DmvrArgs &a, hipStream_t s);
void launch_dbk(xgpu_ctx *c, const DbkArgs &a, int dir, const DevPic &src, const DevPic &dst, bool order_rl = false);
void upload_transform_tables(const int *tm, const int16_t *ats, hipStream_t s);
int  itdq_group_size(int log2w, int log2h);
void launch_addb_fused(xgpu_ctx *c, const AddbArgs &a, const DevPic &src, const DevPic &dst);
void launch_alf(xgpu_ctx *c, const AlfArgs &a, const AddbArgs *deblock, const DevPic &src, const DevPic &dst);
void launch_pad(xgpu_ctx *c, const DevPic &p);
void launch_copy_bw(xgpu_ctx *c, const void *src, void *dst, size_t bytes);
void launch_output(xgpu_ctx *c, const DevPic &pic, const int32_t *d_dra, int out_bd, int crop_l, int crop_r, int crop_t, int crop_b, uint8_t *d_dst, bool raw16 = false,
                   hipStream_t s = nullptr);
struct RgbOutArgs {
    const int16_t *y, *u, *v;
    int      sy, sc;
    int      w, h, cw, ch;
    uint8_t *dst;
    size_t   pitch, plane;
    int      aligned;
    int      bgr;
    int      coef[5], shift;
    float    fcoef[5];
    int      yo, co, maxv;
    int      hc;
    int      ve[2], vo[2];
    const int32_t *dra;
};
void launch_output_rgb(const RgbOutArgs &a, int layout, int dtype, int upsample, hipStream_t s);
void launch_output_yuv444(const RgbOutArgs &a, int layout, int dtype, int upsample, hipStream_t s);
struct CmParams {
    const float *lin, *tone, *enc;
    int      n_lin, use_matrix;
    float    m[9], luma[3], scale;
    float    outmax;
};
struct CmOutArgs : RgbOutArgs { CmParams cm; };
static inline size_t cm_table_floats(int n_lin, bool tone, bool enc) { return (size_t)n_lin + (tone ? XGPU_CM_CURVE_SIZE : 0) + (enc ? XGPU_CM_CURVE_SIZE : 0); }
void launch_output_cm(const CmOutArgs &a, int layout, int dtype, int upsample, hipStream_t s);
struct ScaleTaps { const int32_t *first, *count; const int16_t *w; int stride; };
struct ScaledOutArgs : RgbOutArgs {
    int      dw, dh;
    ScaleTaps yl, yc;
    ScaleTaps xl, xc;
    uint16_t *mid;
    int      mpy, mpc;
    int      smax;
    int      capy, capc;
    int      normalize;
    float    mean[3], inv_std[3];
};
void launch_output_scaled(const ScaledOutArgs &a, int layout, int dtype, hipStream_t s);
void launch_scale_vertical(const ScaledOutArgs &a, hipStream_t s);
int  scale_build_tables(int ws, int hs, int wd, int hd, int filter, int chroma_loc, std::vector<uint8_t> &blob, ScaleTabs &tb, int x_off = 0);
struct __attribute__((aligned(16))) RoiDesc {
    uint64_t dst;
    int      x, y, w, h;
    int      ix, iy, iw, ih;
    uint32_t mid;
    int      mpy, mpc;
    uint32_t first[4], count[4], wt[4];
    int      stride[4];
    int      skip;
    int      pad_[2];
};
static_assert(sizeof(RoiDesc) == 128, "RoiDesc must be 128 bytes");
struct RoisOutArgs : ScaledOutArgs {
    const uint8_t *blk;
    int      n;
    float    padv[3];
};
void launch_output_rois(const RoisOutArgs &a, int layout, int dtype, int max_w, int max_ih, hipStream_t s);
void launch_rois_vertical(const RoisOutArgs &a, int max_w, int max_ih, hipStream_t s);
struct ScaledCmOutArgs : ScaledOutArgs { CmParams cm; };
struct RoisCmOutArgs : RoisOutArgs { CmParams cm; };
void launch_output_scaled_cm(const ScaledCmOutArgs &a, int layout, int dtype, hipStream_t s);
void launch_output_rois_cm(const RoisCmOutArgs &a, int layout, int dtype, int max_w, int max_ih, hipStream_t s);
void launch_output_scaled_lin(const ScaledCmOutArgs &a, int layout, int dtype, int upsample, hipStream_t s);
void launch_output_rois_lin(const RoisCmOutArgs &a, int layout, int dtype, int upsample, int max_w, int max_ih, hipStream_t s);
static const size_t LIN_LDS_LIMIT = 64 * 1024;
int  scale_build_axis(int n, int s, int h, int N, int S, int H, int filter, bool transposed, int group, std::vector<uint8_t> &blob, ScaleAxisTab &t, int *cap);
struct __attribute__((aligned(16))) LadderDesc {
    uint64_t dst;
    uint64_t pitch;
    uint32_t mid[2];
    int      mp;
    int      plane;
    int      sw;
    int      rows, cols;
    int      pair;
    uint32_t first, count, wt;
    int      stride;
};
static_assert(sizeof(LadderDesc) == 64, "LadderDesc must be 64 bytes");
#define LADDER_GROUP 4
struct LadderOutArgs : ScaledOutArgs {
    const uint8_t *blk;
    int      n, nh;
    int      cap;
    int      cshift, cmaxv, cout8, clsh;
};
void launch_output_ladder(const LadderOutArgs &a, int dtype, int max_sw, int max_vrows, int max_cols, int max_rows, hipStream_t s);
struct RoisPrepArgs {
    uint8_t *blk;
    const void *boxes;
    const int *count;
    xgpu_roi_result *results;
    int      capacity, box_format;
    int      pw, ph, mw, mh;
    int      wd, hd, fit, filter, chroma_loc;
    int      capy, capc;
    size_t   image_pitch;
    uint32_t tab, slot;
    uint32_t off_first[4], off_count[4], off_w[4];
    uint32_t mid_slot;
};
void launch_rois_prepare(const RoisPrepArgs &a, hipStream_t s);
struct WarpOutArgs : ScaledOutArgs {
    const int64_t *maps;
    int32_t *status;
    int      n;
    int      ls;
    int      border;
    int      sh, sv;
    float    padv[3];
    size_t   image_pitch;
};
void launch_output_warp(const WarpOutArgs &a, int layout, int dtype, hipStream_t s);
struct RemapOutArgs : ScaledOutArgs {
    const uint8_t *grid;
    size_t   grid_pitch;
    int      gw, gh;
    int      k;
    int      f32;
    int      n;
    int      ls;
    int      border;
    int      sh, sv;
    float    padv[3];
    size_t   image_pitch;
};
void launch_output_remap(const RemapOutArgs &a, int layout, int dtype, hipStream_t s);
void launch_test_scale_taps(int n_plane, int subsampling, int siting, int n_dst, int filter, int32_t *first, int32_t *count, int16_t *w, int w_stride, hipStream_t s);
struct SemiPlanarArgs {
    const int16_t *y, *u, *v;
    int      sy, sc;
    int      w, ch;
    uint8_t *dst;
    size_t   pitch, chroma_off;
    int      aligned;
// ... 84 lines not shown
```

### xevd_amd/csrc/xgpu_shims.hip

```cpp
#include "xgpu_host.h"

static int test_mc(xgpu_ctx *c, const int16_t *plane, int pw, int ph, int ref_x, int ref_y, int has_dx, int has_dy,
                   int gmv_x, int gmv_y, int16_t *pred, int w, int h, int bd, int luma)
{
    ARGCHK(c, c != NULL); ARGCHK(c, plane && pred && pw > 0 && ph > 0 && w > 0 && h > 0);
    ARGCHK(c, luma ? ((w & 3) == 0 && (h & 3) == 0) : ((w & 1) == 0 && (h & 1) == 0));
    int16_t *dp = NULL, *dq = NULL;
    const size_t pb = sizeof(int16_t) * (size_t)pw * ph + 64, qb = sizeof(int16_t) * (size_t)w * h;
    HIPCHK(c, hipMalloc((void **)&dp, pb));
    HIPCHK(c, hipMalloc((void **)&dq, qb));
    HIPCHK(c, hipMemcpyAsync(dp, plane, pb - 64, hipMemcpyHostToDevice, c->stream));
    launch_test_mc(c, dp, pw, ref_x, ref_y, has_dx, has_dy, gmv_x, gmv_y, dq, w, h, bd, luma);
    HIPCHK(c, hipMemcpyAsync(pred, dq, qb, hipMemcpyDeviceToHost, c->stream));
    HIPCHK(c, hipStreamSynchronize(c->stream));
    (void)hipFree(dp); (void)hipFree(dq);
    return XGPU_OK;
}
int xgpu_test_mc_l(xgpu_ctx *c, const int16_t *plane, int pw, int ph, int ref_x, int ref_y, int has_dx, int has_dy,
                   int gmv_x, int gmv_y, int16_t *pred, int w, int h, int bd)
{ return test_mc(c, plane, pw, ph, ref_x, ref_y, has_dx, has_dy, gmv_x, gmv_y, pred, w, h, bd, 1); }
int xgpu_test_mc_c(xgpu_ctx *c, const int16_t *plane, int pw, int ph, int ref_x, int ref_y, int has_dx, int has_dy,
                   int gmv_x, int gmv_y, int16_t *pred, int w, int h, int bd)
{ return test_mc(c, plane, pw, ph, ref_x, ref_y, has_dx, has_dy, gmv_x, gmv_y, pred, w, h, bd, 0); }

int xgpu_test_recon(xgpu_ctx *c, const int16_t *coef, const int16_t *pred, int is_coef, int cuw, int cuh, int s_rec, int16_t *rec, int bit_depth)
{
    ARGCHK(c, c != NULL); ARGCHK(c, coef && pred && rec && cuw >= 2 && cuh >= 1 && !(cuw & 1) && cuw <= 128 && cuh <= 128 && s_rec >= cuw && bit_depth >= 8 && bit_depth <= 12);
    const size_t nb = sizeof(int16_t) * (size_t)cuw * cuh, rb = sizeof(int16_t) * (size_t)s_rec * cuh;
    int16_t *d = NULL;
    HIPCHK(c, hipMalloc((void **)&d, 2 * nb + rb));
    int16_t *dc = d, *dp = d + (size_t)cuw * cuh, *dr = dp + (size_t)cuw * cuh;
    HIPCHK(c, hipMemcpyAsync(dc, coef, nb, hipMemcpyHostToDevice, c->stream));
    HIPCHK(c, hipMemcpyAsync(dp, pred, nb, hipMemcpyHostToDevice, c->stream));
    HIPCHK(c, hipMemcpyAsync(dr, rec, rb, hipMemcpyHostToDevice, c->stream));
    launch_test_recon(c, dc, dp, is_coef, cuw, cuh, dr, s_rec, bit_depth);
    HIPCHK(c, hipMemcpyAsync(rec, dr, rb, hipMemcpyDeviceToHost, c->stream));
    HIPCHK(c, hipStreamSynchronize(c->stream));
    (void)hipFree(d);
    return XGPU_OK;
}
static int test_dbk(xgpu_ctx *c, int16_t *plane, int16_t *plane_v, int pw, int ph, int x, int y, int st, int st_v, int hor, int bd, int chroma)
{
    ARGCHK(c, c != NULL); ARGCHK(c, plane && (!chroma || plane_v) && pw > 0 && ph > 0 && bd >= 8 && bd <= 12 && st >= 0 && st_v >= 0);
    const int len = chroma ? 2 : 4;
    ARGCHK(c, hor ? (y >= 2 && y + 2 <= ph && x >= 0 && x + len <= pw) : (x >= 2 && x + 2 <= pw && y >= 0 && y + len <= ph));
    const size_t nb = sizeof(int16_t) * (size_t)pw * ph;
    int16_t *d = NULL;
    HIPCHK(c, hipMalloc((void **)&d, 2 * nb));
    HIPCHK(c, hipMemcpyAsync(d, plane, nb, hipMemcpyHostToDevice, c->stream));
    if (chroma) HIPCHK(c, hipMemcpyAsync(d + (size_t)pw * ph, plane_v, nb, hipMemcpyHostToDevice, c->stream));
    launch_test_dbk(c, d + (size_t)y * pw + x, d + (size_t)pw * ph + (size_t)y * pw + x, st, st_v, pw, bd, hor, chroma);
    HIPCHK(c, hipMemcpyAsync(plane, d, nb, hipMemcpyDeviceToHost, c->stream));
    if (chroma) HIPCHK(c, hipMemcpyAsync(plane_v, d + (size_t)pw * ph, nb, hipMemcpyDeviceToHost, c->stream));
    HIPCHK(c, hipStreamSynchronize(c->stream));
    (void)hipFree(d);
    return XGPU_OK;
}
int xgpu_test_dbk(xgpu_ctx *c, int16_t *plane, int pw, int ph, int x, int y, int st, int hor, int bit_depth)
{ return test_dbk(c, plane, NULL, pw, ph, x, y, st, 0, hor, bit_depth, 0); }
int xgpu_test_dbk_chroma(xgpu_ctx *c, int16_t *u, int16_t *v, int pw, int ph, int x, int y, int st_u, int st_v, int hor, int bit_depth)
{ return test_dbk(c, u, v, pw, ph, x, y, st_u, st_v, hor, bit_depth, 1); }

int xgpu_test_batch_resid(xgpu_ctx *c, xgpu_dbatch *db, int16_t *resid)
{
    ARGCHK(c, c != NULL); ARGCHK(c, db != NULL && resid != NULL);
    if (db->n_coef) HIPCHK(c, hipMemcpyAsync(resid, db->d_resid, sizeof(int16_t) * db->n_coef, hipMemcpyDeviceToHost, c->stream));
    HIPCHK(c, hipStreamSynchronize(c->stream));
    return XGPU_OK;
}

int xgpu_test_itdq_ex(xgpu_ctx *c, int16_t *coef, int n_blocks, int log2w, int log2h, const uint8_t *qp, int bit_depth, int tr_v, int tr_h, int log2s)
{
    ARGCHK(c, c != NULL); ARGCHK(c, coef && qp && n_blocks > 0 && log2w >= 1 && log2w <= 6 && log2h >= 1 && log2h <= 6 && bit_depth >= 8 && bit_depth <= 16);
    ARGCHK(c, tr_v >= TR_DCT2 && tr_v <= TR_DCT8 && tr_h >= TR_DCT2 && tr_h <= TR_DCT8);
    ARGCHK(c, (tr_v == TR_DCT2 && tr_h == TR_DCT2) || (tr_v != TR_DCT2 && tr_h != TR_DCT2 && log2w >= 2 && log2w <= 5 && log2h >= 2 && log2h <= 5));
    ARGCHK(c, log2s >= log2w && log2s <= 12 && (log2s == log2w || (log2w >= 3 && log2w + log2h > 4)));
    const size_t per = (size_t)1 << (log2s + log2h), nb = per * n_blocks * sizeof(int16_t);
    ARGCHK(c, per * n_blocks <= 0x7FFFFFFFu);
    std::vector<TbRec> tbs(n_blocks);
    std::vector<TbWave> wv;
    for (int i = 0; i < n_blocks; i++) { tbs[i].off = (uint32_t)(per * i); tbs[i].log2w = (uint8_t)log2w; tbs[i].log2h = (uint8_t)log2h; tbs[i].qp = qp[i]; tbs[i].log2s = (uint8_t)log2s; }
    const int pw = itdq_group_size(log2w, log2h);
    for (int f = 0; f < n_blocks; f += pw)
        wv.push_back({ (uint32_t)f, (uint16_t)std::min(pw, n_blocks - f), (uint8_t)log2w, (uint8_t)log2h, (uint8_t)tr_v, (uint8_t)tr_h, { 0, 0 } });
    int16_t *dc = NULL, *dr = NULL; TbRec *dt = NULL; TbWave *dw = NULL;
    HIPCHK(c, hipMalloc((void **)&dc, nb)); HIPCHK(c, hipMalloc((void **)&dr, nb));
    HIPCHK(c, hipMalloc((void **)&dt, sizeof(TbRec) * tbs.size())); HIPCHK(c, hipMalloc((void **)&dw, sizeof(TbWave) * wv.size()));
    HIPCHK(c, hipMemcpyAsync(dc, coef, nb, hipMemcpyHostToDevice, c->stream));
    if (log2s != log2w) HIPCHK(c, hipMemcpyAsync(dr, coef, nb, hipMemcpyHostToDevice, c->stream));
    HIPCHK(c, hipMemcpyAsync(dt, tbs.data(), sizeof(TbRec) * tbs.size(), hipMemcpyHostToDevice, c->stream));
    HIPCHK(c, hipMemcpyAsync(dw, wv.data(), sizeof(TbWave) * wv.size(), hipMemcpyHostToDevice, c->stream));
    ItdqArgs ia; ia.coef = dc; ia.resid = dr; ia.tbs = dt; ia.waves = dw; ia.n_waves = (int)wv.size(); ia.bd = bit_depth; ia.iqt = c->sp.tool_iqt;
    launch_itdq(c, ia, c->stream);
    HIPCHK(c, hipMemcpyAsync(coef, dr, nb, hipMemcpyDeviceToHost, c->stream));
    HIPCHK(c, hipStreamSynchronize(c->stream));
    (void)hipFree(dc); (void)hipFree(dr); (void)hipFree(dt); (void)hipFree(dw);
    return XGPU_OK;
}
int xgpu_test_itdq(xgpu_ctx *c, int16_t *coef, int n_blocks, int log2w, int log2h, const uint8_t *qp, int bit_depth)
{ return xgpu_test_itdq_ex(c, coef, n_blocks, log2w, log2h, qp, bit_depth, TR_DCT2, TR_DCT2, log2w); }

int xgpu_test_scale_taps_device(xgpu_ctx *c, int n_plane, int subsampling, int siting_half_luma, int n_dst, int filter, int32_t *first, int32_t *count, int16_t *w,
                                int w_stride)
{
    ARGCHK(c, c != NULL);
    const int widest = xgpu_scale_taps(n_plane, subsampling, siting_half_luma, n_dst, filter, first, count, NULL, 0);
    if (widest < 0) return widest;
    ARGCHK(c, !w || w_stride >= widest);
    const size_t ib = sizeof(int32_t) * (size_t)n_dst, wb = w ? sizeof(int16_t) * (size_t)n_dst * w_stride : 0;
    uint8_t *d = NULL;
    HIPCHK(c, hipSetDevice(c->sp.device));
    HIPCHK(c, hipMalloc((void **)&d, 2 * ib + wb + 16));
    HIPCHK(c, hipMemsetAsync(d, 0xFF, 2 * ib + wb, c->stream));
    int32_t *df = (int32_t *)d, *dc = df + n_dst;
    int16_t *dw = w ? (int16_t *)(dc + n_dst) : NULL;
    launch_test_scale_taps(n_plane, subsampling, siting_half_luma, n_dst, filter, df, dc, dw, w_stride, c->stream);
    HIPCHK(c, hipMemcpyAsync(first, df, ib, hipMemcpyDeviceToHost, c->stream));
    HIPCHK(c, hipMemcpyAsync(count, dc, ib, hipMemcpyDeviceToHost, c->stream));
    if (w) HIPCHK(c, hipMemcpyAsync(w, dw, wb, hipMemcpyDeviceToHost, c->stream));
    HIPCHK(c, hipStreamSynchronize(c->stream));
    (void)hipFree(d);
    int wide = 0;
    for (int o = 0; o < n_dst; o++) wide = count[o] > wide ? count[o] : wide;
    return wide;
}
```

### xevd_amd/decoder.py

```python
import ctypes as C

import numpy as np

from . import abi


_DTYPE_CODES = {}


def _codes(*names):
    codes = _DTYPE_CODES.get(names)
    if codes is None:
        import torch
        every = {"uint8": abi.OUT_U8, "int16": abi.OUT_U16, "uint16": abi.OUT_U16, "float16": abi.OUT_F16, "bfloat16": abi.OUT_BF16, "float32": abi.OUT_F32}
        codes = _DTYPE_CODES[names] = {getattr(torch, n): every[n] for n in (names or every) if getattr(torch, n, None) is not None}
    return codes


def _out_tensor(out, shape, dtype, dev):
    if out is None:
        import torch
        out = torch.empty(shape, dtype=dtype, device=dev)
    if out.device != dev or out.dtype != dtype or out.shape != tuple(shape):
        raise ValueError(f"out: expected {tuple(shape)} {dtype} on {dev}, got {tuple(out.shape)} {out.dtype} on {out.device}")
# ... 709 lines not shown
    def pic_output_wait(self, ticket):
        self._chk(self.lib.xgpu_pic_output_wait(self.ctx, ticket), "xgpu_pic_output_wait")

    def batch_dmvr_mvs(self, h):
        n = self._chk(self.lib.xgpu_batch_dmvr_mvs(self.ctx, h, None, 0), "xgpu_batch_dmvr_mvs")
        out = np.zeros((max(n, 1), 2, 2), np.int16)
        self._chk(self.lib.xgpu_batch_dmvr_mvs(self.ctx, h, out.ctypes.data, n), "xgpu_batch_dmvr_mvs")
        return out[:n]

    def batch_info(self, h):
        v = (C.c_int * 8)()
        self._chk(self.lib.xgpu_batch_info(self.ctx, h, v), "xgpu_batch_info")
        return dict(zip(("n_cu", "n_tb", "itdq_items", "dep_nodes", "dep_nodes_level1", "dep_levels", "dmvr_sub_blocks", "affine_tiles"), list(v)))

    def batch_wait_upload(self, h):
        self._chk(self.lib.xgpu_batch_wait_upload(self.ctx, h), "xgpu_batch_wait_upload")

    def pic_upload_padded(self, pic, bufs):
        y, u, v = (np.ascontiguousarray(p, np.int16) for p in bufs)
        self._chk(self.lib.xgpu_pic_upload_padded(self.ctx, pic, y.ctypes.data, u.ctypes.data, v.ctypes.data), "xgpu_pic_upload_padded")

    def pic_download_padded(self, pic):
        y = np.zeros((self.height + 2 * abi.PAD_L, self.width + 2 * abi.PAD_L), np.int16)
        u = np.zeros((self.height // 2 + 2 * abi.PAD_C, self.width // 2 + 2 * abi.PAD_C), np.int16)
        v = np.zeros_like(u)
        self._chk(self.lib.xgpu_pic_download_padded(self.ctx, pic, y.ctypes.data, u.ctypes.data, v.ctypes.data), "xgpu_pic_download_padded")
        return [y, u, v]

    def pic_download_padded_luma(self, pic):
        y = np.zeros((self.height + 2 * abi.PAD_L, self.width + 2 * abi.PAD_L), np.int16)
        self._chk(self.lib.xgpu_pic_download_padded(self.ctx, pic, y.ctypes.data, None, None), "xgpu_pic_download_padded")
        return y

    def frame_begin(self, pic, poc, refs, qp_u_offset=0, qp_v_offset=0, deblock_on=0, alf_on=0, alpha_off=0, beta_off=0):
        fp = abi.FrameParams()
        fp.pic, fp.poc = pic, poc
        for l in range(2):
            idxs = [i for (i, ll) in refs if ll == l]
            fp.num_refp[l] = (max(idxs) + 1) if idxs else 0
        for (i, l), (slot, rpoc) in refs.items():
            fp.refp_pic[i][l] = slot
            fp.refp_poc[i][l] = rpoc
        fp.qp_u_offset, fp.qp_v_offset = qp_u_offset, qp_v_offset
        fp.deblock_alpha_offset, fp.deblock_beta_offset = alpha_off, beta_off
        fp.deblock_on, fp.alf_on = int(deblock_on), int(alf_on)
        self._chk(self.lib.xgpu_frame_begin(self.ctx, C.byref(fp)), "xgpu_frame_begin")

    def batch_create(self, batch):
        cb, keep = abi.make_cu_batch(batch)
        h = C.c_void_p()
        self._chk(self.lib.xgpu_batch_create(self.ctx, C.byref(cb), C.byref(h)), "xgpu_batch_create")
        self._batches.append(h)
        return h

    def batch_create_from_struct(self, cu_batch):
        h = C.c_void_p()
        self._chk(self.lib.xgpu_batch_create(self.ctx, C.byref(cu_batch), C.byref(h)), "xgpu_batch_create")
        self._batches.append(h)
        return h

    def batch_resid(self, h, n_coef):
        out = np.zeros(max(n_coef, 1), np.int16)
        self._chk(self.lib.xgpu_test_batch_resid(self.ctx, h, out.ctypes.data), "xgpu_test_batch_resid")
        return out

    def batch_destroy(self, h):
        self._batches = [b for b in self._batches if b.value != h.value]
        self.lib.xgpu_batch_destroy(self.ctx, h)

    def batch_prepare(self, h):
        self._chk(self.lib.xgpu_batch_prepare(self.ctx, h), "xgpu_batch_prepare")

    def batch_recon(self, h, next_batch=None):
        if next_batch is None:
            self._chk(self.lib.xgpu_batch_recon(self.ctx, h), "xgpu_batch_recon")
        else:
            self._chk(self.lib.xgpu_batch_recon_ahead(self.ctx, h, next_batch), "xgpu_batch_recon_ahead")

    def deblock(self):
        self._chk(self.lib.xgpu_deblock(self.ctx), "xgpu_deblock")

    def alf(self, params):
        ap, keep = abi.make_alf_params(params)
        self._chk(self.lib.xgpu_alf(self.ctx, C.byref(ap)), "xgpu_alf")

    def pad(self):
        self._chk(self.lib.xgpu_pad(self.ctx), "xgpu_pad")

    def frame_end(self):
        self._chk(self.lib.xgpu_frame_end(self.ctx), "xgpu_frame_end")

    def decode_picture(self, pic, poc, refs, batch_handle, deblock=True, pad=True, qp_u_offset=0, qp_v_offset=0,
                       alpha_off=0, beta_off=0, alf=None, next_batch=None):
        self.frame_begin(pic, poc, refs, qp_u_offset, qp_v_offset, deblock_on=deblock, alf_on=alf is not None,
                         alpha_off=alpha_off, beta_off=beta_off)
        self.batch_recon(batch_handle, next_batch)
        if deblock:
            self.deblock()
        if alf is not None:
            self.alf(alf)
        if pad:
            self.pad()
        self.frame_end()

    def timing_enable(self, on=True):
        self._chk(self.lib.xgpu_timing_enable(self.ctx, 1 if on else 0), "xgpu_timing_enable")

    def timing_reset(self):
        self._chk(self.lib.xgpu_timing_reset(self.ctx), "xgpu_timing_reset")

    def timing_get(self):
        ms = (C.c_double * abi.K_COUNT)()
        n = (C.c_longlong * abi.K_COUNT)()
        self._chk(self.lib.xgpu_timing_get(self.ctx, ms, n), "xgpu_timing_get")
        return {abi.K_NAMES[i]: (ms[i], n[i]) for i in range(abi.K_COUNT)}

    def measure_copy_bw(self, nbytes=1 << 30, iters=10):
        g = C.c_double()
        self._chk(self.lib.xgpu_measure_copy_bw(self.ctx, nbytes, iters, C.byref(g)), "xgpu_measure_copy_bw")
        return g.value

    def test_mc(self, plane, ref_x, ref_y, has_dx, has_dy, gmv_x, gmv_y, w, h, bit_depth, luma=True):
        plane = np.ascontiguousarray(plane, np.int16)
        pred = np.zeros((h, w), np.int16)
        fn = self.lib.xgpu_test_mc_l if luma else self.lib.xgpu_test_mc_c
        self._chk(fn(self.ctx, plane.ctypes.data, plane.shape[1], plane.shape[0], ref_x, ref_y, has_dx, has_dy, gmv_x, gmv_y,
                     pred.ctypes.data, w, h, bit_depth), "xgpu_test_mc")
        return pred

    def test_recon(self, coef, pred, is_coef, rec, bit_depth):
        coef, pred = np.ascontiguousarray(coef, np.int16), np.ascontiguousarray(pred, np.int16)
        rec = np.ascontiguousarray(rec, np.int16).copy()
        self._chk(self.lib.xgpu_test_recon(self.ctx, coef.ctypes.data, pred.ctypes.data, int(is_coef), pred.shape[1], pred.shape[0], rec.shape[1],
                                           rec.ctypes.data, bit_depth), "xgpu_test_recon")
        return rec

    def test_dbk(self, plane, x, y, st, hor, bit_depth, plane_v=None, st_v=0):
        plane = np.ascontiguousarray(plane, np.int16).copy()
        if plane_v is None:
            self._chk(self.lib.xgpu_test_dbk(self.ctx, plane.ctypes.data, plane.shape[1], plane.shape[0], x, y, st, int(hor), bit_depth), "xgpu_test_dbk")
            return plane
        plane_v = np.ascontiguousarray(plane_v, np.int16).copy()
        self._chk(self.lib.xgpu_test_dbk_chroma(self.ctx, plane.ctypes.data, plane_v.ctypes.data, plane.shape[1], plane.shape[0], x, y, st, st_v, int(hor),
                                                bit_depth), "xgpu_test_dbk_chroma")
        return plane, plane_v

    def test_itdq(self, coef, log2w, log2h, qp, bit_depth, tr_v=0, tr_h=0, log2s=None):
        coef = np.ascontiguousarray(coef, np.int16).copy()
        qp = np.ascontiguousarray(qp, np.uint8)
        log2s = log2w if log2s is None else log2s
        assert coef.size == len(qp) << (log2s + log2h), "n blocks of h << log2s samples"
        self._chk(self.lib.xgpu_test_itdq_ex(self.ctx, coef.ctypes.data, len(qp), log2w, log2h, qp.ctypes.data, bit_depth, tr_v, tr_h, log2s), "xgpu_test_itdq_ex")
        return coef
```

Before: 3428 frames/s.

## Process pairs of ITDQ waves per workgroup when wave count is large

Templates the ITDQ small and item paths on an item count so one workgroup can handle two same-class transform waves at once, sharing matrix row loads and loop control across both. It issues both items' coefficient loads before the dependent math to overlap memory latency, and gives each item its own LDS region and mask slots. The fused intra+itdq launch packs two itdq items per workgroup when the wave count exceeds a threshold (env-tunable, default 4096) and changes the span ratio. This trades higher LDS and register pressure, which can lower occupancy, for fewer workgroups and better latency hiding. Test entry points for the paired path are also added.

```diff
diff --git a/include/xevd_hip.h b/include/xevd_hip.h
--- a/include/xevd_hip.h
+++ b/include/xevd_hip.h
@@ -374,6 +374,8 @@
 int xgpu_test_build_batch(const xgpu_seq_params *sp, const xgpu_cu_batch *b, int threads, uint64_t digest[XGPU_TEST_BUILD_DIGESTS], int info[XGPU_BATCH_INFO_COUNT], double *ms);
 int xgpu_test_itdq(xgpu_ctx *ctx, int16_t *coef, int n_blocks, int log2w, int log2h, const uint8_t *qp, int bit_depth);
 int xgpu_test_itdq_ex(xgpu_ctx *ctx, int16_t *coef, int n_blocks, int log2w, int log2h, const uint8_t *qp, int bit_depth, int tr_v, int tr_h, int log2s);
+int xgpu_test_itdq_pairs(xgpu_ctx *ctx, int16_t *coef, int n_blocks, int log2w, int log2h, const uint8_t *qp, int bit_depth, int tr_v, int tr_h, int log2s);
+int xgpu_test_itdq_pairs_mixed(xgpu_ctx *ctx, int16_t *coef, int n_groups, const int32_t *groups, const uint8_t *qp, int bit_depth);
 int xgpu_test_scale_taps_device(xgpu_ctx *ctx, int n_plane, int subsampling, int siting_half_luma, int n_dst, int filter, int32_t *first, int32_t *count,
                                 int16_t *w, int w_stride);
 
diff --git a/xevd_amd/abi.py b/xevd_amd/abi.py
--- a/xevd_amd/abi.py
+++ b/xevd_amd/abi.py
@@ -737,6 +737,8 @@
     "xgpu_test_dbk_chroma": (C.c_int, [C.c_void_p, C.c_void_p, C.c_void_p] + [C.c_int] * 8),
     "xgpu_test_itdq": (C.c_int, [C.c_void_p, C.c_void_p, C.c_int, C.c_int, C.c_int, C.c_void_p, C.c_int]),
     "xgpu_test_itdq_ex": (C.c_int, [C.c_void_p, C.c_void_p, C.c_int, C.c_int, C.c_int, C.c_void_p, C.c_int, C.c_int, C.c_int, C.c_int]),
+    "xgpu_test_itdq_pairs": (C.c_int, [C.c_void_p, C.c_void_p, C.c_int, C.c_int, C.c_int, C.c_void_p, C.c_int, C.c_int, C.c_int, C.c_int]),
+    "xgpu_test_itdq_pairs_mixed": (C.c_int, [C.c_void_p, C.c_void_p, C.c_int, C.c_void_p, C.c_void_p, C.c_int]),
     "xgpu_test_scale_taps_device": (C.c_int, [C.c_void_p] + [C.c_int] * 5 + [C.POINTER(C.c_int32), C.POINTER(C.c_int32), C.POINTER(C.c_int16), C.c_int]),
 }
 
diff --git a/xevd_amd/csrc/itdq_body.h b/xevd_amd/csrc/itdq_body.h
--- a/xevd_amd/csrc/itdq_body.h
+++ b/xevd_amd/csrc/itdq_body.h
@@ -111,28 +111,24 @@
     return (uint32_t)__builtin_amdgcn_readfirstlane((int)m);
 }
 
+template <int N, bool PIN>
+__device__ __forceinline__ void itq_row(uint32_t (&rw)[N], const uint32_t *row)
+{
+#pragma unroll
+    for (int n = 0; n < N; n++) rw[n] = row[n];
+    if constexpr (PIN) {
+#pragma unroll
+        for (int n = 0; n < N; n++) asm volatile("" : "+s"(rw[n]));
+    }
+}
+
 template <int L>
 __device__ __forceinline__ const uint32_t *itdq_matrix(int tr) { return (tr == TR_DCT2 || L < 2 || L > 5) ? k_tmp + tmp_base(L) : k_atsp[tr - 1] + atsp_base(L); }
 
 template <int LW, int LH, bool IQT>
-__device__ __forceinline__ void itdq_small(const ItdqArgs &a, const TbWave wv)
+__device__ __forceinline__ void itdq_small_tb(const ItdqArgs &a, const itq_v2 rec, const uint32_t (&raw)[(1 << (LW + LH)) / 2], const uint32_t *tmh, const uint32_t *tmw, bool s16_mid)
 {
     constexpr int W = 1 << LW, H = 1 << LH, S = W * H;
-    static_assert(S <= 16 && itdq_group(LW, LH) <= 256, "one TB per lane");
-    const int p = threadIdx.x;
-    if (p >= wv.count) return;
-    const itq_v2 rec = *(const itq_v2_u *)(a.tbs + wv.first + p);
-    const uint32_t *tmh = itdq_matrix<LH>(wv.tr_v), *tmw = itdq_matrix<LW>(wv.tr_h);
-    const bool s16_mid = IQT || wv.tr_v != TR_DCT2 || wv.tr_h != TR_DCT2;
-    uint32_t raw[S / 2];
-    if constexpr (S == 4) { const itq_v2 v = *(const itq_v2_s *)(a.coef + rec.x); raw[0] = v.x; raw[1] = v.y; }
-    else {
-#pragma unroll
-        for (int i = 0; i < S / 8; i++) {
-            const itq_v4 v = *(const itq_v4_u *)(a.coef + rec.x + 8 * i);
-            raw[4 * i] = v.x; raw[4 * i + 1] = v.y; raw[4 * i + 2] = v.z; raw[4 * i + 3] = v.w;
-        }
-    }
     const ItdqScale<(LW + LH) & 1, IQT> dq(rec_qp(rec), a.bd, LW + LH);
     int d[S];
 #pragma unroll
@@ -210,9 +206,54 @@
     }
 }
 
-template <int LW, int LH, bool IQT>
-__device__ __forceinline__ void itdq_item(const ItdqArgs &a, const TbWave wv, uint32_t *lds, uint32_t *s_tb)
-{
+template <int LW, int LH, bool IQT, int NI = 1>
+__device__ __forceinline__ void itdq_small(const ItdqArgs &a, const TbWave (&wv)[NI], const int tid)
+{
+    constexpr int W = 1 << LW, H = 1 << LH, S = W * H;
+    static_assert(S <= 16 && itdq_group(LW, LH) <= 256, "one TB per lane");
+    static_assert(NI == 1 || NI == 2, "an item, or a pair of one class and one transform pair");
+    const int p = tid;
+    bool live[NI], any = false;
+#pragma unroll
+    for (int i = 0; i < NI; i++) { live[i] = p < wv[i].count; any |= live[i]; }
+    if (!any) return;
+    itq_v2 rec[NI];
+#pragma unroll
+    for (int i = 0; i < NI; i++) { rec[i] = itq_any<itq_v2>(); itq_rec_if(rec[i], a.tbs + wv[i].first + p, live[i]); }
+    const uint32_t *tmh = itdq_matrix<LH>(wv[0].tr_v), *tmw = itdq_matrix<LW>(wv[0].tr_h);
+    const bool s16_mid = IQT || wv[0].tr_v != TR_DCT2 || wv[0].tr_h != TR_DCT2;
+    constexpr int NV = S == 4 ? 1 : S / 8;
+    typedef typename std::conditional<S == 4, itq_v2, itq_v4>::type cvec;
+    cvec cv[NI][NV];
+    if (NI > 1) __builtin_amdgcn_s_waitcnt(0x0F70);
+#pragma unroll
+    for (int i = 0; i < NI; i++) {
+#pragma unroll
+        for (int k = 0; k < NV; k++) cv[i][k] = itq_any<cvec>();
+        if (live[i]) {
+            if constexpr (S == 4) cv[i][0] = *(const itq_v2_s *)(a.coef + rec[i].x);
+            else {
+#pragma unroll
+                for (int k = 0; k < NV; k++) cv[i][k] = *(const itq_v4_u *)(a.coef + rec[i].x + 8 * k);
+            }
+        }
+    }
+#pragma unroll
+    for (int i = 0; i < NI; i++) {
+        if (!live[i]) continue;
+        uint32_t raw[S / 2];
+#pragma unroll
+        for (int k = 0; k < S / 2; k++) raw[k] = cv[i][k / (S == 4 ? 2 : 4)][k % (S == 4 ? 2 : 4)];
+        itdq_small_tb<LW, LH, IQT>(a, rec[i], raw, tmh, tmw, s16_mid);
+    }
+}
+
+template <bool IQT> constexpr int itdq_item_dwords() { return IQT ? ITDQ_LDS_DWORDS - ITDQ_PLANES_DWORDS / 2 : ITDQ_LDS_DWORDS; }
+template <int LW, int LH, bool IQT, int NI = 1>
+__device__ __forceinline__ void itdq_item(const ItdqArgs &a, const TbWave (&wv)[NI], uint32_t *lds, uint32_t *s_tb, const int tid)
+{
+    static_assert(NI == 1 || NI == 2, "an item, or a pair of one class and one transform pair");
+    constexpr int ITEM = itdq_item_dwords<IQT>();
     constexpr int W = 1 << LW, H = 1 << LH;
     constexpr int N1 = H > 16 ? 16 : H, C1 = H / N1;
     constexpr int N2 = W > 16 ? 16 : W, C2 = W / N2;
@@ -223,193 +264,288 @@
     static_assert(2 * PLANE <= ITDQ_PLANES_DWORDS && G * W * H <= 4096 && G <= ITDQ_MAX_G, "LDS budget");
     constexpr int PLANES_DWORDS = IQT ? ITDQ_PLANES_DWORDS / 2 : ITDQ_PLANES_DWORDS;
     constexpr bool RMASK = H >= 16, CMASK = W >= 16;
-    uint32_t *s_rm = s_tb, *s_cm = s_tb + ITDQ_MAX_G, *s_rec = s_tb + 2 * ITDQ_MAX_G;
-    const int t = threadIdx.x;
+    uint32_t *s_rm[NI], *s_cm[NI], *s_rec[NI];
+#pragma unroll
+    for (int i = 0; i < NI; i++) { s_rm[i] = s_tb + i * ITDQ_TB_DWORDS; s_cm[i] = s_rm[i] + ITDQ_MAX_G; s_rec[i] = s_rm[i] + 2 * ITDQ_MAX_G; }
+    const int t = tid;
 
     constexpr int S = W * H, UN = S >= 8 ? 8 : 4, NU = G * S / UN, NR = (NU + 255) / 256;
     typedef typename std::conditional<UN == 8, itq_v4, itq_v2>::type cvec;
-    bool on[NR];
+    bool on[NI][NR];
     int up[NR], uo[NR];
-    itq_v2 rec[NR];
+    itq_v2 rec[NI][NR];
 #pragma unroll
     for (int r = 0; r < NR; r++) {
         const int u = t + 256 * r;
         up[r] = (u * UN) / S; uo[r] = (u * UN) % S;
-        on[r] = (NU % 256 == 0 || u < NU) && up[r] < wv.count;
-        rec[r] = itq_any<itq_v2>();
-        itq_rec_if(rec[r], a.tbs + wv.first + up[r], on[r]);
+#pragma unroll
+        for (int i = 0; i < NI; i++) {
+            on[i][r] = (NU % 256 == 0 || u < NU) && up[r] < wv[i].count;
+            rec[i][r] = itq_any<itq_v2>();
+            itq_rec_if(rec[i][r], a.tbs + wv[i].first + up[r], on[i][r]);
+        }
     }
     if (RMASK || CMASK) {
-        if (t < G) { s_rm[t] = 0; s_cm[t] = 0; }
+        if (t < G) {
+#pragma unroll
+            for (int i = 0; i < NI; i++) { s_rm[i][t] = 0; s_cm[i][t] = 0; }
+        }
         __syncthreads();
     }
-    const uint32_t *tmh = itdq_matrix<LH>(wv.tr_v), *tmw = itdq_matrix<LW>(wv.tr_h);
-    const bool s16_mid = IQT || wv.tr_v != TR_DCT2 || wv.tr_h != TR_DCT2;
+    const uint32_t *tmh = itdq_matrix<LH>(wv[0].tr_v), *tmw = itdq_matrix<LW>(wv[0].tr_h);
+    const bool s16_mid = IQT || wv[0].tr_v != TR_DCT2 || wv[0].tr_h != TR_DCT2;
     asm volatile("" :: "s"(tmh), "s"(tmw));
-    int16_t *ldsh = (int16_t *)lds;
-    int16_t *ldsl = (int16_t *)(lds + PLANE);
-    uint32_t *ldsc = lds + PLANES_DWORDS;
-    cvec cv[NR];
-#pragma unroll
-    for (int r = 0; r < NR; r++) {
-        cv[r] = itq_any<cvec>();
-        if (on[r]) {
-            const int16_t *src = a.coef + rec[r].x + ((uo[r] >> LW) << rec_log2s(rec[r])) + (uo[r] & (W - 1));
-            if constexpr (UN == 8) cv[r] = *(const itq_v4_u *)src; else cv[r] = *(const itq_v2_s *)src;
-        }
-    }
-#pragma unroll
-    for (int r = 0; r < NR; r++) {
-        if (!on[r]) continue;
-        const int p = up[r], o = uo[r];
-        const ItdqScale<(LW + LH) & 1, IQT> dq(rec_qp(rec[r]), a.bd, LW + LH);
-        if (o == 0) { s_rec[2 * p] = rec[r].x; s_rec[2 * p + 1] = rec[r].y; }
-        uint32_t raw[UN / 2];
-#pragma unroll
-        for (int i = 0; i < UN / 2; i++) raw[i] = cv[r][i];
-#pragma unroll
-        for (int i = 0; i < UN / 2; i++) {
-            if (raw[i] == 0) continue;
-            raw[i] = pack16(dq((int16_t)(raw[i] & 0xFFFF)), dq((int16_t)(raw[i] >> 16)));
-            if (RMASK) atomicOr(&s_rm[p], 1u << ((o + 2 * i) >> (LW + 1)));
-            if (CMASK) atomicOr(&s_cm[p], 1u << (((o + 2 * i) & (W - 1)) >> 1));
-        }
-#pragma unroll
-        for (int i = 0; i < UN / 2; i++) ldsc[(p * S + o) / 2 + i] = raw[i];
+    cvec cv[NI][NR];
+    if (NI > 1) __builtin_amdgcn_s_waitcnt(0x0F70);
+#pragma unroll
+    for (int i = 0; i < NI; i++) {
+#pragma unroll
+        for (int r = 0; r < NR; r++) {
+            cv[i][r] = itq_any<cvec>();
+            if (on[i][r]) {
+                const int16_t *src = a.coef + rec[i][r].x + ((uo[r] >> LW) << rec_log2s(rec[i][r])) + (uo[r] & (W - 1));
+                if constexpr (UN == 8) cv[i][r] = *(const itq_v4_u *)src; else cv[i][r] = *(const itq_v2_s *)src;
+            }
+        }
+    }
+#pragma unroll
+    for (int i = 0; i < NI; i++) {
+        uint32_t *ldsc = lds + i * ITEM + PLANES_DWORDS;
+#pragma unroll
+        for (int r = 0; r < NR; r++) {
+            if (!on[i][r]) continue;
+            const int p = up[r], o = uo[r];
+            const ItdqScale<(LW + LH) & 1, IQT> dq(rec_qp(rec[i][r]), a.bd, LW + LH);
+            if (o == 0) { s_rec[i][2 * p] = rec[i][r].x; s_rec[i][2 * p + 1] = rec[i][r].y; }
+            uint32_t raw[UN / 2];
+#pragma unroll
+            for (int k = 0; k < UN / 2; k++) raw[k] = cv[i][r][k];
+#pragma unroll
+            for (int k = 0; k < UN / 2; k++) {
+                if (raw[k] == 0) continue;
+                raw[k] = pack16(dq((int16_t)(raw[k] & 0xFFFF)), dq((int16_t)(raw[k] >> 16)));
+                if (RMASK) atomicOr(&s_rm[i][p], 1u << ((o + 2 * k) >> (LW + 1)));
+                if (CMASK) atomicOr(&s_cm[i][p], 1u << (((o + 2 * k) & (W - 1)) >> 1));
+            }
+#pragma unroll
+            for (int k = 0; k < UN / 2; k++) ldsc[(p * S + o) / 2 + k] = raw[k];
+        }
     }
     __syncthreads();
 
-    uint32_t rows1 = 0;
-    if (RMASK) rows1 = wave_masks<G, LW>(s_rm, t);
+    uint32_t rows1[NI], rows1_any = 0;
+#pragma unroll
+    for (int i = 0; i < NI; i++) { rows1[i] = RMASK ? wave_masks<G, LW>(s_rm[i], t) : 0u; rows1_any |= rows1[i]; }
     if (t < G * W * C1) {
         const int idx = t % (G * W);
         int chunk = t / (G * W);
         if (UNI1) chunk = __builtin_amdgcn_readfirstlane(chunk);
         const int p = idx >> LW, j = idx & (W - 1);
-        const bool valid = p < wv.count;
-        const uint32_t vmask = valid ? 0xFFFFFFFFu : 0u;
-        const int16_t *src = (const int16_t *)ldsc + p * (W * H) + j;
-
-        int acc[N1];
-#pragma unroll
-        for (int n = 0; n < N1; n++) acc[n] = 0;
+        bool valid[NI];
+        uint32_t vmask[NI];
+        const int16_t *src[NI];
+        int acc[NI][N1];
+#pragma unroll
+        for (int i = 0; i < NI; i++) {
+            valid[i] = p < wv[i].count;
+            vmask[i] = valid[i] ? 0xFFFFFFFFu : 0u;
+            src[i] = (const int16_t *)(lds + i * ITEM + PLANES_DWORDS) + p * (W * H) + j;
+#pragma unroll
+            for (int n = 0; n < N1; n++) acc[i][n] = 0;
+        }
         if (RMASK) {
-            for (uint32_t m = rows1; m; m &= m - 1) {
+            for (uint32_t m = rows1_any; m; m &= m - 1) {
                 const int k2 = __builtin_ctz(m);
-                const uint32_t vp = pack16(src[(2 * k2) * W], src[(2 * k2 + 1) * W]) & vmask;
-                const uint32_t *row = tmh + k2 * H + chunk * N1;
-#pragma unroll
-                for (int n = 0; n < N1; n++) acc[n] = dot2(row[n], vp, acc[n]);
+                uint32_t vp[NI];
+#pragma unroll
+                for (int i = 0; i < NI; i++) vp[i] = pack16(src[i][(2 * k2) * W], src[i][(2 * k2 + 1) * W]) & vmask[i];
+                uint32_t row[N1];
+                itq_row<N1, (NI > 1 && UNI1)>(row, tmh + k2 * H + chunk * N1);
+#pragma unroll
+                for (int i = 0; i < NI; i++) {
+                    if (NI > 1 && !((rows1[i] >> k2) & 1)) continue;
+#pragma unroll
+                    for (int n = 0; n < N1; n++) acc[i][n] = dot2(row[n], vp[i], acc[i][n]);
+                }
             }
         } else {
             for (int k2 = 0; k2 < H / 2; k2++) {
-                const uint32_t vp = pack16(src[(2 * k2) * W], src[(2 * k2 + 1) * W]) & vmask;
-                if (__ballot(vp != 0) == 0) continue;
-                const uint32_t *row = tmh + k2 * H + chunk * N1;
-#pragma unroll
-                for (int n = 0; n < N1; n++) acc[n] = dot2(row[n], vp, acc[n]);
+                uint32_t vp[NI];
+                bool go[NI], any = false;
+#pragma unroll
+                for (int i = 0; i < NI; i++) {
+                    vp[i] = pack16(src[i][(2 * k2) * W], src[i][(2 * k2 + 1) * W]) & vmask[i];
+                    go[i] = __ballot(vp[i] != 0) != 0;
+                    any |= go[i];
+                }
+                if (!any) continue;
+                uint32_t row[N1];
+                itq_row<N1, (NI > 1 && UNI1)>(row, tmh + k2 * H + chunk * N1);
+#pragma unroll
+                for (int i = 0; i < NI; i++) {
+                    if (NI > 1 && !go[i]) continue;
+#pragma unroll
+                    for (int n = 0; n < N1; n++) acc[i][n] = dot2(row[n], vp[i], acc[i][n]);
+                }
             }
         }
         const int base = (p * H + chunk * N1) * (2 * RS) + j;
-        if (CMASK && !(valid && ((s_cm[p] >> (j >> 1)) & 1))) {
-        } else if (s16_mid) {
-#pragma unroll
-            for (int n = 0; n < N1; n++) ldsh[base + n * (2 * RS)] = (int16_t)clip16((acc[n] + 64) >> 7);
-        } else {
-#pragma unroll
-            for (int n = 0; n < N1; n++) {
-                ldsh[base + n * (2 * RS)] = (int16_t)(acc[n] >> 15);
-                ldsl[base + n * (2 * RS)] = (int16_t)(acc[n] & 0x7FFF);
+#pragma unroll
+        for (int i = 0; i < NI; i++) {
+            int16_t *ldsh = (int16_t *)(lds + i * ITEM);
+            int16_t *ldsl = (int16_t *)(lds + i * ITEM + PLANE);
+            if (CMASK && !(valid[i] && ((s_cm[i][p] >> (j >> 1)) & 1))) {
+            } else if (s16_mid) {
+#pragma unroll
+                for (int n = 0; n < N1; n++) ldsh[base + n * (2 * RS)] = (int16_t)clip16((acc[i][n] + 64) >> 7);
+            } else {
+#pragma unroll
+                for (int n = 0; n < N1; n++) {
+                    ldsh[base + n * (2 * RS)] = (int16_t)(acc[i][n] >> 15);
+                    ldsl[base + n * (2 * RS)] = (int16_t)(acc[i][n] & 0x7FFF);
+                }
             }
         }
     }
     __syncthreads();
 
-    uint32_t cols2 = 0;
-    if (CMASK) cols2 = wave_masks<G, LH>(s_cm, t);
+    uint32_t cols2[NI], cols2_any = 0;
+#pragma unroll
+    for (int i = 0; i < NI; i++) { cols2[i] = CMASK ? wave_masks<G, LH>(s_cm[i], t) : 0u; cols2_any |= cols2[i]; }
     if (t < G * H * C2) {
         const int idx = t % (G * H);
         int chunk = t / (G * H);
         if (UNI2) chunk = __builtin_amdgcn_readfirstlane(chunk);
         const int p = idx >> LH, r = idx & (H - 1);
-        if (p >= wv.count) return;
-        const uint32_t own = CMASK ? s_cm[p] : 0xFFFFFFFFu;
-        itq_v2 tb;
-        tb.x = s_rec[2 * p]; tb.y = s_rec[2 * p + 1];
+        bool live[NI], any_live = false;
+#pragma unroll
+        for (int i = 0; i < NI; i++) { live[i] = p < wv[i].count; any_live |= live[i]; }
+        if (!any_live) return;
+        uint32_t own[NI];
+        itq_v2 tb[NI];
+        const uint32_t *inh[NI], *inl[NI];
+#pragma unroll
+        for (int i = 0; i < NI; i++) {
+            own[i] = CMASK ? s_cm[i][p] : 0xFFFFFFFFu;
+            if (NI > 1 && !live[i]) own[i] = 0;
+            tb[i].x = s_rec[i][2 * p]; tb[i].y = s_rec[i][2 * p + 1];
+            inh[i] = lds + i * ITEM + (p * H + r) * RS;
+            inl[i] = inh[i] + PLANE;
+        }
         const int shift2 = s16_mid ? 12 - (a.bd - 8) : 7 + 12 - (a.bd - 8);
-        const uint32_t *inh = lds + (p * H + r) * RS;
-        const uint32_t *inl = inh + PLANE;
-        int res[N2];
+        int res[NI][N2];
         if (s16_mid) {
-            int s[N2];
-#pragma unroll
-            for (int n = 0; n < N2; n++) s[n] = 1 << (shift2 - 1);
+            int s[NI][N2];
+#pragma unroll
+            for (int i = 0; i < NI; i++)
+#pragma unroll
+                for (int n = 0; n < N2; n++) s[i][n] = 1 << (shift2 - 1);
             if (CMASK) {
-                for (uint32_t m = cols2; m; m &= m - 1) {
+                for (uint32_t m = cols2_any; m; m &= m - 1) {
                     const int k2 = __builtin_ctz(m);
-                    const uint32_t vp = inh[k2] & (0u - ((own >> k2) & 1));
-                    const uint32_t *row = tmw + k2 * W + chunk * N2;
-#pragma unroll
-                    for (int n = 0; n < N2; n++) s[n] = dot2(row[n], vp, s[n]);
+                    uint32_t vp[NI];
+#pragma unroll
+                    for (int i = 0; i < NI; i++) vp[i] = inh[i][k2] & (0u - ((own[i] >> k2) & 1));
+                    uint32_t row[N2];
+                    itq_row<N2, (NI > 1 && UNI2)>(row, tmw + k2 * W + chunk * N2);
+#pragma unroll
+                    for (int i = 0; i < NI; i++) {
+                        if (NI > 1 && !((cols2[i] >> k2) & 1)) continue;
+#pragma unroll
+                        for (int n = 0; n < N2; n++) s[i][n] = dot2(row[n], vp[i], s[i][n]);
+                    }
                 }
             } else {
                 for (int k2 = 0; k2 < W / 2; k2++) {
-                    const uint32_t vp = inh[k2];
-                    if (__ballot(vp != 0) == 0) continue;
+                    uint32_t vp[NI];
+                    bool go[NI], any = false;
+#pragma unroll
+                    for (int i = 0; i < NI; i++) {
+                        vp[i] = inh[i][k2] & (0u - ((own[i] >> k2) & 1));
+                        go[i] = __ballot(vp[i] != 0) != 0;
+                        any |= go[i];
+                    }
+                    if (!any) continue;
+                    uint32_t row[N2];
+                    itq_row<N2, (NI > 1 && UNI2)>(row, tmw + k2 * W + chunk * N2);
+#pragma unroll
+                    for (int i = 0; i < NI; i++) {
+                        if (NI > 1 && !go[i]) continue;
+#pragma unroll
+                        for (int n = 0; n < N2; n++) s[i][n] = dot2(row[n], vp[i], s[i][n]);
+                    }
+                }
+            }
+#pragma unroll
+            for (int i = 0; i < NI; i++)
+#pragma unroll
+                for (int n = 0; n < N2; n++) res[i][n] = clip16(s[i][n] >> shift2);
+        } else {
+            int sh[NI][N2], sl[NI][N2];
+#pragma unroll
+            for (int i = 0; i < NI; i++)
+#pragma unroll
+                for (int n = 0; n < N2; n++) { sh[i][n] = 0; sl[i][n] = 0; }
+            if (CMASK) {
+                for (uint32_t m = cols2_any; m; m &= m - 1) {
+                    const int k2 = __builtin_ctz(m);
                     const uint32_t *row = tmw + k2 * W + chunk * N2;
 #pragma unroll
-                    for (int n = 0; n < N2; n++) s[n] = dot2(row[n], vp, s[n]);
-                }
-            }
-#pragma unroll
-            for (int n = 0; n < N2; n++) res[n] = clip16(s[n] >> shift2);
-        } else {
-            int sh[N2], sl[N2];
-#pragma unroll
-            for (int n = 0; n < N2; n++) { sh[n] = 0; sl[n] = 0; }
-            if (CMASK) {
-                for (uint32_t m = cols2; m; m &= m - 1) {
-                    const int k2 = __builtin_ctz(m);
-                    const uint32_t mine = 0u - ((own >> k2) & 1);
-                    const uint32_t vh = inh[k2] & mine, vl = inl[k2] & mine;
-                    const uint32_t *row = tmw + k2 * W + chunk * N2;
-#pragma unroll
-                    for (int n = 0; n < N2; n++) { sh[n] = dot2(row[n], vh, sh[n]); sl[n] = dot2(row[n], vl, sl[n]); }
+                    for (int i = 0; i < NI; i++) {
+                        const uint32_t mine = 0u - ((own[i] >> k2) & 1);
+                        const uint32_t vh = inh[i][k2] & mine, vl = inl[i][k2] & mine;
+#pragma unroll
+                        for (int n = 0; n < N2; n++) { sh[i][n] = dot2(row[n], vh, sh[i][n]); sl[i][n] = dot2(row[n], vl, sl[i][n]); }
+                    }
                 }
             } else {
                 for (int k2 = 0; k2 < W / 2; k2++) {
-                    const uint32_t vh = inh[k2], vl = inl[k2];
-                    if (__ballot((vh | vl) != 0) == 0) continue;
+                    uint32_t vh[NI], vl[NI], nz = 0;
+#pragma unroll
+                    for (int i = 0; i < NI; i++) {
+                        const uint32_t mine = 0u - ((own[i] >> k2) & 1);
+                        vh[i] = inh[i][k2] & mine; vl[i] = inl[i][k2] & mine;
+                        nz |= vh[i] | vl[i];
+                    }
+                    if (__ballot(nz != 0) == 0) continue;
                     const uint32_t *row = tmw + k2 * W + chunk * N2;
 #pragma unroll
-                    for (int n = 0; n < N2; n++) { sh[n] = dot2(row[n], vh, sh[n]); sl[n] = dot2(row[n], vl, sl[n]); }
+                    for (int i = 0; i < NI; i++)
+#pragma unroll
+                        for (int n = 0; n < N2; n++) { sh[i][n] = dot2(row[n], vh[i], sh[i][n]); sl[i][n] = dot2(row[n], vl[i], sl[i][n]); }
                 }
             }
             const long long add = 1ll << (shift2 - 1);
 #pragma unroll
-            for (int n = 0; n < N2; n++) {
-                const long long s = (long long)sh[n] * 32768 + sl[n] + add;
-                res[n] = (int)min(max(s >> shift2, -32768ll), 32767ll);
-            }
-        }
-        int16_t *out = a.resid + tb.x + (r << rec_log2s(tb)) + chunk * N2;
-        if constexpr (N2 >= 8) {
-#pragma unroll
-            for (int n = 0; n < N2; n += 8) {
-                uint4 v;
-                v.x = pack16(res[n + 0], res[n + 1]);
-                v.y = pack16(res[n + 2], res[n + 3]);
-                v.z = pack16(res[n + 4], res[n + 5]);
-                v.w = pack16(res[n + 6], res[n + 7]);
-                *(uint4 *)(out + n) = v;
-            }
-        } else if constexpr (N2 == 4) {
-            uint2 v;
-            v.x = pack16(res[0], res[1]);
-            v.y = pack16(res[2], res[3]);
-            *(uint2 *)out = v;
-        } else {
-            *(uint32_t *)out = pack16(res[0], res[1]);
+            for (int i = 0; i < NI; i++)
+#pragma unroll
+                for (int n = 0; n < N2; n++) {
+                    const long long s = (long long)sh[i][n] * 32768 + sl[i][n] + add;
+                    res[i][n] = (int)min(max(s >> shift2, -32768ll), 32767ll);
+                }
+        }
+#pragma unroll
+        for (int i = 0; i < NI; i++) {
+            if (NI > 1 && !live[i]) continue;
+            int16_t *out = a.resid + tb[i].x + (r << rec_log2s(tb[i])) + chunk * N2;
+            if constexpr (N2 >= 8) {
+#pragma unroll
+                for (int n = 0; n < N2; n += 8) {
+                    uint4 v;
+                    v.x = pack16(res[i][n + 0], res[i][n + 1]);
+                    v.y = pack16(res[i][n + 2], res[i][n + 3]);
+                    v.z = pack16(res[i][n + 4], res[i][n + 5]);
+                    v.w = pack16(res[i][n + 6], res[i][n + 7]);
+                    *(uint4 *)(out + n) = v;
+                }
+            } else if constexpr (N2 == 4) {
+                uint2 v;
+                v.x = pack16(res[i][0], res[i][1]);
+                v.y = pack16(res[i][2], res[i][3]);
+                *(uint2 *)out = v;
+            } else {
+                *(uint32_t *)out = pack16(res[i][0], res[i][1]);
+            }
         }
     }
 }
@@ -420,14 +556,51 @@
     static_assert(sizeof(TbWave) == 12 && alignof(TbWave) == 4, "TbWave is read as three dwords");
     const uint32_t *w = (const uint32_t *)(a.waves + wi);
     const uint32_t w0 = w[0], w1 = w[1], w2 = w[2];
-    TbWave wv;
-    wv.first = w0; wv.count = (uint16_t)(w1 & 0xFFFF); wv.log2w = (uint8_t)(w1 >> 16); wv.log2h = (uint8_t)(w1 >> 24); wv.tr_v = (uint8_t)w2; wv.tr_h = (uint8_t)(w2 >> 8);
-#define CASE(lw, lh) case (lw) * 8 + (lh): if constexpr ((lw) + (lh) <= 4) itdq_small<lw, lh, IQT>(a, wv); else itdq_item<lw, lh, IQT>(a, wv, lds, s_tb); break;
+    TbWave wv[1];
+    wv[0].first = w0; wv[0].count = (uint16_t)(w1 & 0xFFFF); wv[0].log2w = (uint8_t)(w1 >> 16); wv[0].log2h = (uint8_t)(w1 >> 24); wv[0].tr_v = (uint8_t)w2; wv[0].tr_h = (uint8_t)(w2 >> 8);
+#define CASE(lw, lh) case (lw) * 8 + (lh): if constexpr ((lw) + (lh) <= 4) itdq_small<lw, lh, IQT>(a, wv, threadIdx.x); else itdq_item<lw, lh, IQT>(a, wv, lds, s_tb, threadIdx.x); break;
 #define ROW(lw) CASE(lw, 1) CASE(lw, 2) CASE(lw, 3) CASE(lw, 4) CASE(lw, 5) CASE(lw, 6)
-    switch (wv.log2w * 8 + wv.log2h) {
+    switch (wv[0].log2w * 8 + wv[0].log2h) {
         ROW(1) ROW(2) ROW(3) ROW(4) ROW(5) ROW(6)
         default: break;
     }
 #undef ROW
 #undef CASE
 }
+
+template <bool IQT>
+__device__ __forceinline__ void itdq_dispatch_pair(const ItdqArgs &a, int e0, int n, uint32_t *lds, uint32_t *s_tb)
+{
+    const bool two = n == 2 && e0 + 1 < a.n_waves;
+    const uint32_t *w = (const uint32_t *)(a.waves + e0), *x = (const uint32_t *)(a.waves + e0 + (two ? 1 : 0));
+    const uint32_t w0 = w[0], w1 = w[1], w2 = w[2], x0 = x[0], x1 = x[1], x2 = x[2];
+    TbWave wv[2];
+    wv[0].first = w0; wv[0].count = (uint16_t)(w1 & 0xFFFF); wv[0].log2w = (uint8_t)(w1 >> 16); wv[0].log2h = (uint8_t)(w1 >> 24); wv[0].tr_v = (uint8_t)w2; wv[0].tr_h = (uint8_t)(w2 >> 8);
+    wv[1].first = x0; wv[1].count = (uint16_t)(x1 & 0xFFFF); wv[1].log2w = (uint8_t)(x1 >> 16); wv[1].log2h = (uint8_t)(x1 >> 24); wv[1].tr_v = (uint8_t)x2; wv[1].tr_h = (uint8_t)(x2 >> 8);
+#define ROW(lw) CASE(lw, 1) CASE(lw, 2) CASE(lw, 3) CASE(lw, 4) CASE(lw, 5) CASE(lw, 6)
+    if (two && (w1 >> 16) == (x1 >> 16) && (w2 & 0xFFFFu) == (x2 & 0xFFFFu)) {
+#define CASE(lw, lh) case (lw) * 8 + (lh): if constexpr ((lw) + (lh) <= 4) itdq_small<lw, lh, IQT, 2>(a, wv, threadIdx.x); else itdq_item<lw, lh, IQT, 2>(a, wv, lds, s_tb, threadIdx.x); break;
+        switch (wv[0].log2w * 8 + wv[0].log2h) {
+            ROW(1) ROW(2) ROW(3) ROW(4) ROW(5) ROW(6)
+            default: break;
+        }
+#undef CASE
+        return;
+    }
+#pragma unroll 1
+    for (int k = 0; k < (two ? 2 : 1); k++) {
+        TbWave one[1];
+        one[0] = k ? wv[1] : wv[0];
+        int t = threadIdx.x;
+        asm volatile("" : "+v"(t));
+        __builtin_assume(t >= 0 && t < 256);
+        uint32_t *lds_k = lds + k * itdq_item_dwords<IQT>(), *s_tb_k = s_tb + k * ITDQ_TB_DWORDS;
+#define CASE(lw, lh) case (lw) * 8 + (lh): if constexpr ((lw) + (lh) <= 4) itdq_small<lw, lh, IQT>(a, one, t); else itdq_item<lw, lh, IQT>(a, one, lds_k, s_tb_k, t); break;
+        switch (one[0].log2w * 8 + one[0].log2h) {
+            ROW(1) ROW(2) ROW(3) ROW(4) ROW(5) ROW(6)
+            default: break;
+        }
+#undef CASE
+    }
+#undef ROW
+}
diff --git a/xevd_amd/csrc/k_intra.hip b/xevd_amd/csrc/k_intra.hip
--- a/xevd_amd/csrc/k_intra.hip
+++ b/xevd_amd/csrc/k_intra.hip
@@ -638,19 +638,41 @@
 }
 
 #define FUSED_WAVES 4
+#ifndef ITDQ_PAIRS
+#define ITDQ_PAIRS 1
+#endif
+#ifndef FUSED_SPAN_PCT
+#define FUSED_SPAN_PCT 50
+#endif
+constexpr int fused_items(bool iqt) { return iqt && ITDQ_PAIRS ? 2 : 1; }
 template <int EIPD, bool IBC, bool IQT>
-__global__ __launch_bounds__(64 * FUSED_WAVES) void k_intra_itdq(const IntraArgs a, const ItdqArgs r, uint32_t n_intra_wg, uint64_t rate)
+__global__ __launch_bounds__(64 * FUSED_WAVES) void k_intra_itdq(const IntraArgs a, const ItdqArgs r, uint32_t n_intra_wg, uint64_t rate, uint32_t per_wg)
 {
-    constexpr int ITDQ_DW = (IQT ? ITDQ_LDS_DWORDS - ITDQ_PLANES_DWORDS / 2 : ITDQ_LDS_DWORDS) + ITDQ_TB_DWORDS, INTRA_DW = (FUSED_WAVES * IntraLds<false>::WAVE + 1) / 2 + 4;
+    constexpr int NI = fused_items(IQT);
+    constexpr int ITDQ_DW = NI * (itdq_item_dwords<IQT>() + ITDQ_TB_DWORDS), INTRA_DW = (FUSED_WAVES * IntraLds<false>::WAVE + 1) / 2 + 4;
+    static_assert(!IQT || 4 * ITDQ_DW <= 40 * 1024, "four workgroups per CU in 160 KB of LDS");
     __shared__ __attribute__((aligned(16))) uint32_t raw[ITDQ_DW > INTRA_DW ? ITDQ_DW : INTRA_DW];
     const uint32_t before = min(n_intra_wg, (uint32_t)(((uint64_t)blockIdx.x * rate) >> 32)), after = min(n_intra_wg, (uint32_t)(((uint64_t)(blockIdx.x + 1) * rate) >> 32));
     if (after > before) {
         intra_body<true, EIPD, IBC, false, FUSED_WAVES>(a, blockIdx.x, (int16_t *)raw, raw + INTRA_DW - 1);
     } else {
         const int wi = (int)(blockIdx.x - before);
-        if (wi >= r.n_waves) return;
-        itdq_dispatch<IQT>(r, wi, raw, raw + ITDQ_DW - ITDQ_TB_DWORDS);
-    }
+        if (wi >= (r.n_waves + (int)per_wg - 1) / (int)per_wg) return;
+        if constexpr (NI == 2) itdq_dispatch_pair<IQT>(r, wi * (int)per_wg, (int)per_wg, raw, raw + ITDQ_DW - 2 * ITDQ_TB_DWORDS);
+        else itdq_dispatch<IQT>(r, wi, raw, raw + ITDQ_DW - ITDQ_TB_DWORDS);
+    }
+}
+
+__global__ __launch_bounds__(256) void k_itdq_pairs(const ItdqArgs a)
+{
+    __shared__ __attribute__((aligned(16))) uint32_t raw[2 * (itdq_item_dwords<true>() + ITDQ_TB_DWORDS)];
+    const int pi = blockIdx.x;
+    if (pi >= (a.n_waves + 1) / 2) return;
+    itdq_dispatch_pair<true>(a, 2 * pi, 2, raw, raw + 2 * itdq_item_dwords<true>());
+}
+void launch_itdq_pairs(xgpu_ctx *c, const ItdqArgs &a, hipStream_t s)
+{
+    if (a.n_waves > 0) hipLaunchKernelGGL(k_itdq_pairs, dim3((a.n_waves + 1) / 2), dim3(256), 0, s, a);
 }
 
 void upload_transform_tables_intra(const int *tm, const int16_t *ats, hipStream_t s) { upload_transform_tables_tu(tm, ats, s); }
@@ -662,10 +684,11 @@
     right = right && c->sp.tool_eipd;
     if (next) {
         const uint32_t n_wg = (uint32_t)((a.count + FUSED_WAVES - 1) / FUSED_WAVES);
-        const dim3 g(n_wg + (uint32_t)next->n_waves), b(64 * FUSED_WAVES);
-        const uint32_t span = std::max(n_wg, g.x / 2);
+        const uint32_t per_wg = next->n_waves >= c->itdq_pair_min ? (uint32_t)fused_items(next->iqt != 0) : 1u;
+        const dim3 g(n_wg + ((uint32_t)next->n_waves + per_wg - 1) / per_wg), b(64 * FUSED_WAVES);
+        const uint32_t span = std::max(n_wg, (uint32_t)((uint64_t)g.x * FUSED_SPAN_PCT / 100));
         const uint64_t rate = (((uint64_t)n_wg << 32) + span - 1) / span;
-#define LAUNCHF(E, I) do { if (next->iqt) hipLaunchKernelGGL((k_intra_itdq<E, I, true>), g, b, 0, c->stream, a, *next, n_wg, rate); else hipLaunchKernelGGL((k_intra_itdq<E, I, false>), g, b, 0, c->stream, a, *next, n_wg, rate); } while (0)
+#define LAUNCHF(E, I) do { if (next->iqt) hipLaunchKernelGGL((k_intra_itdq<E, I, true>), g, b, 0, c->stream, a, *next, n_wg, rate, per_wg); else hipLaunchKernelGGL((k_intra_itdq<E, I, false>), g, b, 0, c->stream, a, *next, n_wg, rate, per_wg); } while (0)
         if (right) LAUNCHF(2, true);
         else if (c->sp.tool_eipd) { if (ibc) LAUNCHF(1, true); else LAUNCHF(1, false); }
         else                 { if (ibc) LAUNCHF(0, true); else LAUNCHF(0, false); }
diff --git a/xevd_amd/csrc/xgpu_api.hip b/xevd_amd/csrc/xgpu_api.hip
--- a/xevd_amd/csrc/xgpu_api.hip
+++ b/xevd_amd/csrc/xgpu_api.hip
@@ -110,6 +110,7 @@
     c->builder_threads = 1;
     c->err[0] = 0; c->timing = 0; c->have_frame = 0; c->side_pic = -1; c->d_maps = NULL; c->d_dra = NULL; c->d_cm = NULL; c->cm_tab = NULL; c->d_ctb_flag = NULL; c->stream = 0; c->up_stream = 0; c->down_stream = 0; c->side_stream = 0; c->after_inter = 0; c->have_after_inter = 0; c->where = 0; c->addb_pending = 0;
     c->fork_ev = c->join_ev = 0;
+    c->itdq_pair_min = getenv("XEVD_HIP_ITDQ_PAIR_MIN") ? std::max(1, atoi(getenv("XEVD_HIP_ITDQ_PAIR_MIN"))) : 4096;
     c->intra_small_min = getenv("XEVD_HIP_INTRA_SMALL_MIN") ? std::max(1, atoi(getenv("XEVD_HIP_INTRA_SMALL_MIN"))) : 2048;
     c->addb_scalar = getenv("XEVD_HIP_ADDB_SCALAR") != NULL;
     c->dmvr_scalar = getenv("XEVD_HIP_DMVR_SCALAR") != NULL;
diff --git a/xevd_amd/csrc/xgpu_internal.h b/xevd_amd/csrc/xgpu_internal.h
--- a/xevd_amd/csrc/xgpu_internal.h
+++ b/xevd_amd/csrc/xgpu_internal.h
@@ -336,6 +336,7 @@
     int             pad_done;
     int             where;
     int             order_rl;
+    int             itdq_pair_min;
     int             intra_small_min;
     int             addb_scalar;
     int             dmvr_scalar;
@@ -394,6 +395,7 @@
 };
 
 void launch_itdq(xgpu_ctx *c, const ItdqArgs &a, hipStream_t s);
+void launch_itdq_pairs(xgpu_ctx *c, const ItdqArgs &a, hipStream_t s);
 void launch_inter(xgpu_ctx *c, const InterArgs &a);
 void launch_test_recon(xgpu_ctx *c, const int16_t *coef, const int16_t *pred, int is_coef, int cuw, int cuh, int16_t *rec, int s_rec, int bd);
 void launch_test_dbk(xgpu_ctx *c, int16_t *buf, int16_t *buf_v, int st, int st_v, int stride, int bd, int hor, int chroma);
diff --git a/xevd_amd/csrc/xgpu_shims.hip b/xevd_amd/csrc/xgpu_shims.hip
--- a/xevd_amd/csrc/xgpu_shims.hip
+++ b/xevd_amd/csrc/xgpu_shims.hip
@@ -100,6 +100,53 @@
 int xgpu_test_itdq(xgpu_ctx *c, int16_t *coef, int n_blocks, int log2w, int log2h, const uint8_t *qp, int bit_depth)
 { return xgpu_test_itdq_ex(c, coef, n_blocks, log2w, log2h, qp, bit_depth, TR_DCT2, TR_DCT2, log2w); }
 
+int xgpu_test_itdq_pairs_mixed(xgpu_ctx *c, int16_t *coef, int n_groups, const int32_t *groups, const uint8_t *qp, int bit_depth)
+{
+    ARGCHK(c, c != NULL); ARGCHK(c, coef && groups && qp && n_groups > 0 && bit_depth >= 8 && bit_depth <= 16);
+    ARGCHK(c, c->sp.tool_iqt);
+    std::vector<TbRec> tbs;
+    std::vector<TbWave> wv;
+    size_t total = 0;
+    for (int gi = 0; gi < n_groups; gi++) {
+        const int32_t *g = groups + 6 * gi;
+        const int n_blocks = g[0], log2w = g[1], log2h = g[2], tr_v = g[3], tr_h = g[4], log2s = g[5];
+        ARGCHK(c, n_blocks > 0 && log2w >= 1 && log2w <= 6 && log2h >= 1 && log2h <= 6);
+        ARGCHK(c, tr_v >= TR_DCT2 && tr_v <= TR_DCT8 && tr_h >= TR_DCT2 && tr_h <= TR_DCT8);
+        ARGCHK(c, (tr_v == TR_DCT2 && tr_h == TR_DCT2) || (tr_v != TR_DCT2 && tr_h != TR_DCT2 && log2w >= 2 && log2w <= 5 && log2h >= 2 && log2h <= 5));
+        ARGCHK(c, log2s >= log2w && log2s <= 12 && (log2s == log2w || (log2w >= 3 && log2w + log2h > 4)));
+        const size_t per = (size_t)1 << (log2s + log2h);
+        total = (total + 63) & ~(size_t)63;
+        ARGCHK(c, total + per * n_blocks <= 0x7FFFFFFFu);
+        const int pw = itdq_group_size(log2w, log2h), first = (int)tbs.size();
+        for (int i = 0; i < n_blocks; i++) {
+            TbRec t; t.off = (uint32_t)(total + per * i); t.log2w = (uint8_t)log2w; t.log2h = (uint8_t)log2h; t.qp = qp[first + i]; t.log2s = (uint8_t)log2s;
+            tbs.push_back(t);
+        }
+        for (int f = 0; f < n_blocks; f += pw)
+            wv.push_back({ (uint32_t)(first + f), (uint16_t)std::min(pw, n_blocks - f), (uint8_t)log2w, (uint8_t)log2h, (uint8_t)tr_v, (uint8_t)tr_h, { 0, 0 } });
+        total += per * n_blocks;
+    }
+    const size_t nb = total * sizeof(int16_t);
+    int16_t *dc = NULL, *dr = NULL; TbRec *dt = NULL; TbWave *dw = NULL;
+    HIPCHK(c, hipMalloc((void **)&dc, nb)); HIPCHK(c, hipMalloc((void **)&dr, nb));
+    HIPCHK(c, hipMalloc((void **)&dt, sizeof(TbRec) * tbs.size())); HIPCHK(c, hipMalloc((void **)&dw, sizeof(TbWave) * wv.size()));
+    HIPCHK(c, hipMemcpyAsync(dc, coef, nb, hipMemcpyHostToDevice, c->stream));
+    HIPCHK(c, hipMemsetAsync(dr, 0x5A, nb, c->stream));
+    HIPCHK(c, hipMemcpyAsync(dt, tbs.data(), sizeof(TbRec) * tbs.size(), hipMemcpyHostToDevice, c->stream));
+    HIPCHK(c, hipMemcpyAsync(dw, wv.data(), sizeof(TbWave) * wv.size(), hipMemcpyHostToDevice, c->stream));
+    ItdqArgs ia; ia.coef = dc; ia.resid = dr; ia.tbs = dt; ia.waves = dw; ia.n_waves = (int)wv.size(); ia.bd = bit_depth; ia.iqt = 1;
+    launch_itdq_pairs(c, ia, c->stream);
+    HIPCHK(c, hipMemcpyAsync(coef, dr, nb, hipMemcpyDeviceToHost, c->stream));
+    HIPCHK(c, hipStreamSynchronize(c->stream));
+    (void)hipFree(dc); (void)hipFree(dr); (void)hipFree(dt); (void)hipFree(dw);
+    return XGPU_OK;
+}
+int xgpu_test_itdq_pairs(xgpu_ctx *c, int16_t *coef, int n_blocks, int log2w, int log2h, const uint8_t *qp, int bit_depth, int tr_v, int tr_h, int log2s)
+{
+    const int32_t g[6] = { n_blocks, log2w, log2h, tr_v, tr_h, log2s };
+    return xgpu_test_itdq_pairs_mixed(c, coef, 1, g, qp, bit_depth);
+}
+
 int xgpu_test_scale_taps_device(xgpu_ctx *c, int n_plane, int subsampling, int siting_half_luma, int n_dst, int filter, int32_t *first, int32_t *count, int16_t *w,
                                 int w_stride)
 {
diff --git a/xevd_amd/decoder.py b/xevd_amd/decoder.py
--- a/xevd_amd/decoder.py
+++ b/xevd_amd/decoder.py
@@ -885,3 +885,22 @@
         assert coef.size == len(qp) << (log2s + log2h), "n blocks of h << log2s samples"
         self._chk(self.lib.xgpu_test_itdq_ex(self.ctx, coef.ctypes.data, len(qp), log2w, log2h, qp.ctypes.data, bit_depth, tr_v, tr_h, log2s), "xgpu_test_itdq_ex")
         return coef
+
+    def test_itdq_pairs(self, coef, log2w, log2h, qp, bit_depth, tr_v=0, tr_h=0, log2s=None):
+        coef = np.ascontiguousarray(coef, np.int16).copy()
+        qp = np.ascontiguousarray(qp, np.uint8)
+        log2s = log2w if log2s is None else log2s
+        assert coef.size == len(qp) << (log2s + log2h), "n blocks of h << log2s samples"
+        self._chk(self.lib.xgpu_test_itdq_pairs(self.ctx, coef.ctypes.data, len(qp), log2w, log2h, qp.ctypes.data, bit_depth, tr_v, tr_h, log2s), "xgpu_test_itdq_pairs")
+        return coef
+
+    def test_itdq_pairs_mixed(self, coef, groups, qp, bit_depth):
+        coef = np.ascontiguousarray(coef, np.int16).copy()
+        qp = np.ascontiguousarray(qp, np.uint8)
+        groups = np.ascontiguousarray(groups, np.int32).reshape(-1, 6)
+        total = 0
+        for n, lw, lh, _, _, ls in groups.tolist():
+            total = ((total + 63) & ~63) + (n << (ls + lh))
+        assert coef.size == total and len(qp) == int(groups[:, 0].sum())
+        self._chk(self.lib.xgpu_test_itdq_pairs_mixed(self.ctx, coef.ctypes.data, len(groups), groups.ctypes.data, qp.ctypes.data, bit_depth), "xgpu_test_itdq_pairs_mixed")
+        return coef
```

After: 3491 frames/s (median of 6 runs). 1.8% higher.
